# fredrikekre/PartitionedArrays.jl

Measured on AMD Instinct MI355X. Metric: SpMV+halo GB/s (frac of HBM peak), 3D Poisson 27-pt, 1/2/4/8 MI355X, higher is better.
Workload: dtype f64

## Files before the change

include/pa_hip.h:

```cpp
#ifndef PA_HIP_H
#define PA_HIP_H

#include <stdint.h>

#ifdef __cplusplus
extern "C" {
#endif

enum { PA_F32 = 0, PA_F64 = 1, PA_C64 = 2, PA_C128 = 3 };
enum { PA_REPLACE = 0, PA_ADD = 1 };

typedef struct pa_ctx pa_ctx;
typedef struct pa_index pa_index;
typedef struct pa_xchg pa_xchg;
typedef struct pa_vec pa_vec;
typedef struct pa_mat pa_mat;
typedef struct pa_coo pa_coo;
typedef struct pa_table pa_table;
typedef struct pa_event pa_event;

const char* pa_last_error(void);
int pa_version(void);
int pa_device_count(int* count);
int pa_tune(const char* key, int value, int* previous);
// ... 84 lines not shown
                  int* depth, int* result_flags);
int pa_vec_eval(pa_vec* y, const pa_index* y_idx, const pa_expr* prog, int nvec,
                const pa_vec* const v[], const pa_index* const v_idx[], int nscal,
                const void* scalars, const int* scalar_kinds, int all_lids);
int pa_reduce_expr_all(int n, int kind, const pa_expr* prog, int nvec,
                       const pa_vec* const v[], const pa_index* const v_idx[], int nscal,
                       const void* scalars, const int* scalar_kinds, void* result);

int pa_mat_from_csc(pa_ctx* ctx, int dtype, int index_bytes,
                    int64_t nrows_lids, int64_t ncols_lids,
                    const void* colptr, const void* rowval, const void* nzval,
                    const pa_index* rows, const pa_index* cols,
                    pa_mat** out);
int pa_mat_from_csr(pa_ctx* ctx, int dtype, int index_bytes, int Bi,
                    int64_t nrows_lids, int64_t ncols_lids,
                    const void* rowptr, const void* colval, const void* nzval,
                    const pa_index* rows, const pa_index* cols,
                    pa_mat** out);
int pa_mat_from_coo(pa_ctx* ctx, int dtype, int index_bytes, int ids_global,
                    int64_t nrows_lids, int64_t ncols_lids, int64_t ncoo,
                    const void* I, const void* J, const void* V,
                    const pa_index* rows, const pa_index* cols,
                    int64_t* csc_nnz, int64_t* colptr_out,
                    int64_t* rowval_out, pa_mat** out);
int pa_mat_from_coo_csr(pa_ctx* ctx, int dtype, int index_bytes, int ids_global, int Bi,
                        int64_t nrows_lids, int64_t ncols_lids, int64_t ncoo,
                        const void* I, const void* J, const void* V,
                        const pa_index* rows, const pa_index* cols, int64_t* nnz,
                        int64_t* rowptr_out, int64_t* colval_out, pa_mat** out);
int pa_mat_from_dcoo_csr(const pa_coo* coo, int ids_global, int Bi, int64_t nrows_lids,
                         int64_t ncols_lids, const pa_index* rows, const pa_index* cols,
                         int64_t* nnz, int64_t* rowptr_out, int64_t* colval_out,
                         pa_mat** out);
int pa_coo_create(pa_ctx* ctx, int dtype, int64_t n, const int64_t* I,
                  const int64_t* J, const void* V, pa_coo** out);
int pa_coo_destroy(pa_coo* coo);
int pa_coo_size(const pa_coo* coo, int64_t* n);
int pa_coo_download(const pa_coo* coo, int64_t* I, int64_t* J, void* V);
int pa_coo_assemble_all(int n, pa_coo* const coo[], const pa_index* const rows[],
                        pa_xchg* const rows_xchg[]);
int pa_coo_exchange_all(int n, pa_coo* const coo[], const pa_index* const rows[],
                        pa_xchg* const rows_xchg[]);
int pa_mat_from_dcoo(const pa_coo* coo, int ids_global, int64_t nrows_lids,
                     int64_t ncols_lids, const pa_index* rows,
                     const pa_index* cols, int64_t* csc_nnz,
                     int64_t* colptr_out, int64_t* rowval_out, pa_mat** out);
int pa_mat_set_values(pa_mat* A, const void* nzval);
int pa_mat_fillstored(pa_mat* A, const void* v);
int pa_mat_get_values(const pa_mat* A, void* nzval);
int pa_mat_scatter(pa_mat* A, pa_index* rows, pa_index* cols, int ids_kind,
                   int index_bytes, int op, int on_device, int64_t n,
                   const void* I, const void* J, const void* V);
int pa_mat_gather(const pa_mat* A, pa_index* rows, pa_index* cols, int ids_kind,
                  int index_bytes, int absent_zero, int on_device, int64_t n,
                  const void* I, const void* J, void* out);
int pa_mat_entry_info(const pa_mat* A, int64_t* entries, int64_t* bytes);
#define PA_NZ_OWNED_ROWS 0
#define PA_NZ_ALL_ROWS 1
int pa_mat_findnz(pa_mat* A, pa_index* rows, pa_index* cols, int which_rows, int ids_kind,
                  pa_coo** out);
int pa_mat_xchg_create(pa_mat* A, int32_t n_rcv, const int32_t* parts_rcv,
                       const int32_t* ptrs_rcv, const int64_t* k_rcv,
                       int32_t n_snd, const int32_t* parts_snd,
                       const int32_t* ptrs_snd, const int64_t* k_snd,
                       pa_xchg** out);
int pa_mat_exchange_all(int n, pa_mat* const A[], pa_xchg* const xg[],
                        int op, int reverse, int zero_sent);
int pa_mat_destroy(pa_mat* A);
int pa_mat_info(const pa_mat* A, int64_t* nrows_owned, int64_t* nnz_owned,
                int64_t* slots, int64_t* nslices, int64_t* nslices_interior);
int pa_mat_format_info(const pa_mat* A, int64_t* pattern_slices,
                       int64_t* regular_rows, int64_t* side_rows,
                       int64_t* side_slots);
int pa_mat_delta16_info(const pa_mat* A, int64_t* delta16_slices);
int pa_mat_triple_info(const pa_mat* A, int64_t* t_slices, int64_t* t_rows, int64_t* tri_slices,
                       int64_t* tri_rows);
int pa_mat_pair_info(const pa_mat* A, int64_t* pair_slices, int64_t* pair_rows);

int pa_mat_device_ptrs(const pa_mat* A, uint64_t out[8]);

int pa_mat_traffic(const pa_mat* A, int64_t* value_bytes, int64_t* index_bytes,
                   int64_t* meta_bytes);

int pa_mat_long_rows(const pa_mat* A, int64_t* n_long, int64_t* n_long_nnz);

int pa_spmv_all(int n, pa_mat* const A[], pa_vec* const y[],
                const pa_index* const y_idx[],
                pa_vec* const x[], const pa_index* const x_idx[],
                pa_xchg* const xg[], const void* alpha, const void* beta);

int pa_spmv_dot_all(int n, pa_mat* const A[], pa_vec* const y[],
                    const pa_index* const y_idx[],
                    pa_vec* const x[], const pa_index* const x_idx[],
                    pa_xchg* const xg[], const void* alpha, const void* beta,
                    void* dot_result);
int pa_cg_update_all(int n, pa_vec* const x[], pa_vec* const r[],
                     const pa_vec* const u[], const pa_vec* const c[],
                     const pa_index* const idx[], const void* alpha,
                     double* rnorm);

int pa_mat_diag(const pa_mat* A, const pa_index* rows, const pa_index* cols, pa_vec* d);
int pa_pcg_apply_all(int n, pa_vec* const c[], const pa_vec* const r[], const pa_vec* const d[], const pa_index* const idx[], void* rho);
int pa_pcg_update_all(int n, pa_vec* const x[], pa_vec* const r[], const pa_vec* const u[], pa_vec* const c[], const pa_vec* const d[], const pa_index* const idx[], const void* alpha, double* rnorm, void* rho);

int pa_cg_solve_all(int n, pa_mat* const A[], pa_vec* const x[],
                    const pa_vec* const b[], pa_vec* const u[],
                    pa_vec* const r[], pa_vec* const c[],
                    const pa_index* const idx[], pa_xchg* const xg[],
                    double reltol, double abstol, int64_t maxiter, int batch,
                    int64_t* iterations, double* residual, double* history);

typedef int (*pa_allreduce_max_fn)(float* v, int n, void* user);
int pa_cg_variant_agree(const float local_ms[2], pa_allreduce_max_fn fn, void* user, int* choice);
int pa_cg_fuse_agree(int local_can_fuse, pa_allreduce_max_fn fn, void* user, int* agreed);
int pa_mat_cg_choice(const pa_mat* A, int* choice);

int pa_exchange_all(int n, pa_vec* const v[], pa_xchg* const xg[],
                    const pa_index* const idx[], int op, int reverse,
                    int zero_ghosts);

int pa_exchange_all_async(int n, pa_vec* const v[], pa_xchg* const xg[],
                          const pa_index* const idx[], int op, int reverse,
                          int zero_ghosts, pa_event* const after[],
                          pa_event* done[]);
int pa_mat_exchange_all_async(int n, pa_mat* const A[], pa_xchg* const xg[],
                              int op, int reverse, int zero_sent,
                              pa_event* const after[], pa_event* done[]);
int pa_event_record(pa_ctx* ctx, pa_event** out);
int pa_event_query(const pa_event* ev, int* done);
int pa_event_wait(pa_event* ev);
int pa_ctx_wait_event(pa_ctx* ctx, const pa_event* ev);
int pa_event_destroy(pa_event* ev);

int pa_table_create(pa_ctx* ctx, int dtype, int64_t nrows, const int32_t* ptrs,
                    int ptrs_on_device, pa_table** out);
int pa_table_destroy(pa_table* t);
int pa_table_data(pa_table* t, pa_vec** data);
int pa_table_info(const pa_table* t, int64_t* nrows, int64_t* ndata);
int pa_table_ptrs(const pa_table* t, int32_t* ptrs);
int pa_table_exchange_all(int n, pa_table* const tables[], pa_xchg* const xg[],
                          int op, int reverse, int zero_sent);
int pa_table_exchange_all_async(int n, pa_table* const tables[], pa_xchg* const xg[],
                                int op, int reverse, int zero_sent,
                                pa_event* const after[], pa_event* done[]);

int pa_dot_all(int n, const pa_vec* const a[], const pa_index* const ia[],
               const pa_vec* const b[], const pa_index* const ib[],
               void* result);
int pa_norm2_all(int n, const pa_vec* const a[], const pa_index* const ia[],
                 void* result);
int pa_sum_all(int n, const pa_vec* const a[], const pa_index* const ia[],
               void* result);

int pa_mat_stencil(pa_ctx* ctx, int dtype, int kind, const int64_t gdims[3],
                   const int64_t box_lo[3], const int64_t box_n[3],
                   int64_t nlids_cols, const int32_t* shell_lid,
                   const double* coeffs, int ncoeffs, pa_mat** out);

int pa_ctx_set_timing(pa_ctx* ctx, int enable);
int pa_ctx_kernel_times(pa_ctx* ctx, float* interior_ms, float* halo_ms,
                        float* boundary_ms, int* count);
int pa_ctx_last_kernel_ms(pa_ctx* ctx, float* spmv_interior_ms,
                          float* spmv_boundary_ms);
int pa_ctx_span(pa_ctx* ctx, int stop);
int pa_ctx_span_ms(pa_ctx* ctx, float* ms);

// ... 5 lines not shown
```

partitionedarrays.jl_amd/_lib.py:

```python
from __future__ import annotations

import ctypes as C
import os

import numpy as np

_HERE = os.path.dirname(os.path.abspath(__file__))
LIB_PATH = os.environ.get("PA_HIP_LIB") or os.path.join(_HERE, "libpa_hip.so")

PA_F32, PA_F64, PA_C64, PA_C128 = 0, 1, 2, 3
PA_REPLACE, PA_ADD = 0, 1
TUNE_DROP = -(2 ** 31)
PA_BCAST_F64, PA_BCAST_C128 = 8, 16
PA_IDS_LOCAL, PA_IDS_GLOBAL = 0, 1
PA_SCATTER_ADD, PA_SCATTER_SET = 0, 1
PA_NZ_OWNED_ROWS, PA_NZ_ALL_ROWS = 0, 1

EXPR_MAX_OPS, EXPR_MAX_VECS, EXPR_MAX_SCALARS, EXPR_MAX_DEPTH = 32, 8, 8, 4
(OP_VEC, OP_SCAL, OP_ADD, OP_SUB, OP_MUL, OP_DIV, OP_NEG, OP_ABS, OP_ABS2, OP_CONJ,
 OP_LT, OP_LE, OP_GT, OP_GE, OP_EQ, OP_NE) = range(16)
EXPR_WIDE, EXPR_LREAL, EXPR_RREAL = 1, 2, 4
EXPR_SS, EXPR_SC, EXPR_CS, EXPR_RS = 0, 8, 16, 24
REDUCE_SUM, REDUCE_MAX, REDUCE_MIN = 0, 1, 2

# ... 50 lines not shown
    "pa_vec_upload": [_p, _p, C.c_int64],
    "pa_vec_download": [_p, _p, C.c_int64],
    "pa_vec_device_ptr": [_p, _p],
    "pa_vec_fill": [_p, _p],
    "pa_vec_copy": [_p, _p, _p, _p, C.c_int],
    "pa_vec_axpby": [_p, _p, _p, _p, C.c_int, C.c_int],
    "pa_vec_scatter": [_p, _p, C.c_int, C.c_int, C.c_int, C.c_int, C.c_int, C.c_int64, _p, _p],
    "pa_vec_gather": [_p, _p, C.c_int, C.c_int, C.c_int, C.c_int, C.c_int64, _p, _p],
    "pa_expr_check": [_p, C.c_int, C.c_int, C.c_int, C.POINTER(C.c_int), C.POINTER(C.c_int), C.POINTER(C.c_int)],
    "pa_vec_eval": [_p, _p, _p, C.c_int, C.POINTER(_p), C.POINTER(_p), C.c_int, _p, C.POINTER(C.c_int), C.c_int],
    "pa_reduce_expr_all": [C.c_int, C.c_int, _p, C.c_int, C.POINTER(_p), C.POINTER(_p), C.c_int, _p,
                           C.POINTER(C.c_int), _p],
    "pa_mat_from_csc": [_p, C.c_int, C.c_int, C.c_int64, C.c_int64, _p, _p, _p, _p, _p, C.POINTER(_p)],
    "pa_mat_from_csr": [_p, C.c_int, C.c_int, C.c_int, C.c_int64, C.c_int64, _p, _p, _p, _p, _p, C.POINTER(_p)],
    "pa_coo_create": [_p, C.c_int, C.c_int64, _i64p, _i64p, _p, C.POINTER(_p)],
    "pa_coo_destroy": [_p],
    "pa_coo_size": [_p, _i64p],
    "pa_coo_download": [_p, _i64p, _i64p, _p],
    "pa_coo_assemble_all": [C.c_int, C.POINTER(_p), C.POINTER(_p), C.POINTER(_p)],
    "pa_coo_exchange_all": [C.c_int, C.POINTER(_p), C.POINTER(_p), C.POINTER(_p)],
    "pa_mat_from_dcoo": [_p, C.c_int, C.c_int64, C.c_int64, _p, _p, _i64p, _i64p, _i64p, C.POINTER(_p)],
    "pa_mat_from_coo": [_p, C.c_int, C.c_int, C.c_int, C.c_int64, C.c_int64, C.c_int64, _p, _p, _p, _p, _p, _i64p,
                        _i64p, _i64p, C.POINTER(_p)],
    "pa_mat_from_coo_csr": [_p, C.c_int, C.c_int, C.c_int, C.c_int, C.c_int64, C.c_int64, C.c_int64, _p, _p, _p, _p,
                            _p, _i64p, _i64p, _i64p, C.POINTER(_p)],
    "pa_mat_from_dcoo_csr": [_p, C.c_int, C.c_int, C.c_int64, C.c_int64, _p, _p, _i64p, _i64p, _i64p,
                             C.POINTER(_p)],
    "pa_mat_fillstored": [_p, _p],
    "pa_index_set_gids": [_p, _i64p],
    "pa_add_gids": [_p, C.c_int64, _i64p, C.c_int64, _i64p, _i64p],
    "pa_index_to_lids": [_p, C.c_int64, _i64p],
    "pa_index_to_gids": [_p, C.c_int64, _i64p],
    "pa_mat_findnz": [_p, _p, _p, C.c_int, C.c_int, C.POINTER(_p)],
    "pa_mat_set_values": [_p, _p],
    "pa_mat_get_values": [_p, _p],
    "pa_mat_scatter": [_p, _p, _p, C.c_int, C.c_int, C.c_int, C.c_int, C.c_int64, _p, _p, _p],
    "pa_mat_gather": [_p, _p, _p, C.c_int, C.c_int, C.c_int, C.c_int, C.c_int64, _p, _p, _p],
    "pa_mat_entry_info": [_p, _i64p, _i64p],
    "pa_mat_xchg_create": [_p, C.c_int32, _i32p, _i32p, _i64p, C.c_int32, _i32p, _i32p, _i64p, C.POINTER(_p)],
    "pa_mat_exchange_all": [C.c_int, C.POINTER(_p), C.POINTER(_p), C.c_int, C.c_int, C.c_int],
    "pa_mat_destroy": [_p],
    "pa_mat_info": [_p, _i64p, _i64p, _i64p, _i64p, _i64p],
    "pa_mat_format_info": [_p, _i64p, _i64p, _i64p, _i64p],
    "pa_mat_delta16_info": [_p, _i64p],
    "pa_mat_triple_info": [_p, _i64p, _i64p, _i64p, _i64p],
    "pa_mat_pair_info": [_p, _i64p, _i64p],
    "pa_mat_long_rows": [_p, _i64p, _i64p],
    "pa_mat_stencil": [_p, C.c_int, C.c_int, _i64p, _i64p, _i64p, C.c_int64, _i32p, C.POINTER(C.c_double), C.c_int, C.POINTER(_p)],
    "pa_spmv_all": [C.c_int, C.POINTER(_p), C.POINTER(_p), C.POINTER(_p), C.POINTER(_p), C.POINTER(_p), C.POINTER(_p), _p, _p],
    "pa_spmv_dot_all": [C.c_int, C.POINTER(_p), C.POINTER(_p), C.POINTER(_p), C.POINTER(_p), C.POINTER(_p), C.POINTER(_p), _p, _p, _p],
    "pa_cg_update_all": [C.c_int, C.POINTER(_p), C.POINTER(_p), C.POINTER(_p), C.POINTER(_p), C.POINTER(_p), _p, C.POINTER(C.c_double)],
    "pa_mat_diag": [_p, _p, _p, _p],
    "pa_pcg_apply_all": [C.c_int, C.POINTER(_p), C.POINTER(_p), C.POINTER(_p), C.POINTER(_p), _p],
    "pa_pcg_update_all": [C.c_int, C.POINTER(_p), C.POINTER(_p), C.POINTER(_p), C.POINTER(_p), C.POINTER(_p),
                          C.POINTER(_p), _p, C.POINTER(C.c_double), _p],
    "pa_cg_solve_all": [C.c_int, C.POINTER(_p), C.POINTER(_p), C.POINTER(_p), C.POINTER(_p), C.POINTER(_p),
                        C.POINTER(_p), C.POINTER(_p), C.POINTER(_p), C.c_double, C.c_double, C.c_int64, C.c_int,
                        _i64p, C.POINTER(C.c_double), C.POINTER(C.c_double)],
    "pa_exchange_all": [C.c_int, C.POINTER(_p), C.POINTER(_p), C.POINTER(_p), C.c_int, C.c_int, C.c_int],
    "pa_exchange_all_async": [C.c_int, C.POINTER(_p), C.POINTER(_p), C.POINTER(_p), C.c_int, C.c_int, C.c_int,
                              C.POINTER(_p), C.POINTER(_p)],
    "pa_mat_exchange_all_async": [C.c_int, C.POINTER(_p), C.POINTER(_p), C.c_int, C.c_int, C.c_int, C.POINTER(_p),
                                  C.POINTER(_p)],
    "pa_table_create": [_p, C.c_int, C.c_int64, _p, C.c_int, C.POINTER(_p)],
    "pa_table_destroy": [_p],
    "pa_table_data": [_p, C.POINTER(_p)],
    "pa_table_info": [_p, _i64p, _i64p],
    "pa_table_ptrs": [_p, _i32p],
    "pa_table_exchange_all": [C.c_int, C.POINTER(_p), C.POINTER(_p), C.c_int, C.c_int, C.c_int],
    "pa_table_exchange_all_async": [C.c_int, C.POINTER(_p), C.POINTER(_p), C.c_int, C.c_int, C.c_int, C.POINTER(_p),
                                    C.POINTER(_p)],
    "pa_event_record": [_p, C.POINTER(_p)],
    "pa_event_query": [_p, C.POINTER(C.c_int)],
    "pa_event_wait": [_p],
    "pa_ctx_wait_event": [_p, _p],
    "pa_event_destroy": [_p],
    "pa_dot_all": [C.c_int, C.POINTER(_p), C.POINTER(_p), C.POINTER(_p), C.POINTER(_p), _p],
    "pa_norm2_all": [C.c_int, C.POINTER(_p), C.POINTER(_p), _p],
    "pa_sum_all": [C.c_int, C.POINTER(_p), C.POINTER(_p), _p],
    "pa_ctx_last_kernel_ms": [_p, C.POINTER(C.c_float), C.POINTER(C.c_float)],
    "pa_ctx_kernel_times": [_p, C.POINTER(C.c_float), C.POINTER(C.c_float), C.POINTER(C.c_float),
                            C.POINTER(C.c_int)],
    "pa_mat_traffic": [_p, _i64p, _i64p, _i64p],
    "pa_mat_device_ptrs": [_p, _p],
    "pa_ctx_span": [_p, C.c_int],
    "pa_ctx_span_ms": [_p, C.POINTER(C.c_float)],
    "pa_ctx_set_timing": [_p, C.c_int],
}

EXPORTED = sorted(list(_SIGS) + ["pa_last_error"])


class PAError(RuntimeError):
    pass


def _prepare_runtime():
    try:
        import torch
    except Exception:
        pass


def lib():
    global _lib
    if _lib is not None:
        return _lib
    if not os.path.exists(LIB_PATH):
        raise PAError(f"{LIB_PATH} not built: run `python -c 'import __graft_entry__ as g; g.build()'`")
    _prepare_runtime()
    L = C.CDLL(LIB_PATH)
    for name, args in _SIGS.items():
        if os.environ.get("PA_HIP_LIB") and not hasattr(L, name):
            continue
        f = getattr(L, name)
        f.argtypes = args
        f.restype = C.c_int
    L.pa_last_error.argtypes = []
    L.pa_last_error.restype = C.c_char_p
    _lib = L
    return L


def call(name, *args):
    L = lib()
    rc = getattr(L, name)(*args)
    if rc != 0:
        raise PAError(f"{name}: {L.pa_last_error().decode(errors='replace')}")


def device_count() -> int:
    n = C.c_int(0)
    call("pa_device_count", C.byref(n))
    return n.value


def tune(key: str, value: int) -> int:
    prev = C.c_int(0)
    call("pa_tune", key.encode(), int(value), C.byref(prev))
    return prev.value


def knob_selftest(nthreads: int = 4, iters: int = 2000) -> int:
    n = C.c_int(-1)
    call("pa_knob_selftest", int(nthreads), int(iters), C.byref(n))
    return n.value


ALLREDUCE_MAX_FN = C.CFUNCTYPE(C.c_int, C.POINTER(C.c_float), C.c_int, C.c_void_p)


def cg_variant_agree(local_ms, allreduce_max=None) -> int:
    ms = (C.c_float * 2)(*[float(v) for v in local_ms])
    cb = None
    if allreduce_max is not None:
        def _cb(v, n, _user):
            try:
                out = allreduce_max([v[i] for i in range(n)])
                for i in range(n):
                    v[i] = float(out[i])
                return 0
            except Exception:
                return 1
        cb = ALLREDUCE_MAX_FN(_cb)
    ch = C.c_int(-3)
    call("pa_cg_variant_agree", ms, C.cast(cb, C.c_void_p) if cb else None, None, C.byref(ch))
# ... 52 lines not shown
```

partitionedarrays.jl_amd/csrc/pa_api.cpp:

```cpp
#include <dlfcn.h>
#include <hip/hip_runtime.h>
#include <rccl/rccl.h>

#include <algorithm>
#include <chrono>
#include <cmath>
#include <cstdio>
#include <cstdlib>
#include <cstring>
#include <memory>
#include <numeric>
#include <string>
#include <unordered_map>
#include <atomic>
#include <condition_variable>
#include <functional>
#include <mutex>
#include <thread>
#include <vector>

#include "pa_internal.h"

namespace pa {

static thread_local std::string g_err;
void set_error(const std::string& msg) { g_err = msg; }

void launch_spmv_part(SliceKind kind, const SpmvPart& q, bool has_alpha, int bmode, const void* alpha,
                      const void* beta, hipStream_t st);
void launch_delta16(pa_mat* A, int64_t noids, const int32_t* kind, int32_t* ok, hipStream_t st);
void launch_pattern_detect(pa_mat* A, int64_t noids, int min_pct, int32_t* kind, int32_t* plen, int32_t* pat,
                           uint64_t* mask, int32_t* pghost, int32_t* nirreg, hipStream_t st);
void launch_side_len(pa_mat* A, int64_t n, const int32_t* rows, int32_t* len, int64_t noids,
                     int32_t* sghost, hipStream_t st);
void launch_side_fill(pa_mat* A, const int32_t* rows, const int32_t* len, hipStream_t st);
void launch_fold(int cplx, int nb, const void* in, void* scratch, void* out, unsigned* ticket, hipStream_t st);
void launch_fold_cg_alpha(int dtype, int nb, const void* in, void* scratch, void* out, unsigned* ticket,
                          CGState* cst, hipStream_t st);
void launch_fold_cg_step(int dtype, int nb, const void* in, void* scratch, void* out, unsigned* ticket,
                         CGState* cst, double* history, hipStream_t st);
void launch_cg_xr(int dtype, int64_t n, int64_t noids, const int32_t* own, void* x, void* r, const void* u,
                  const void* c, const void* alpha, const CGState* cst, double* part, int nb, hipStream_t st);
void launch_cg_xu(int dtype, int64_t n, void* x, void* u, const void* r, const CGState* cst, hipStream_t st);
void launch_cg_ghost(int dtype, int64_t lo, int64_t hi, const void* r, const void* uo, void* un, void* x,
                     const CGState* cst, hipStream_t st);
void launch_cg_alpha(int dtype, int P, const void* gathered, CGState* cst, hipStream_t st);
void launch_cg_step(int dtype, int P, const double* gathered, CGState* cst, double* history, hipStream_t st);
void launch_gather_ptrs(int P, const void* const* srcs, int accsz, void* out, hipStream_t st);
void launch_gather_scatter(int P, const void* const* srcs, int accsz, int nd, void* const* dsts, hipStream_t st);
const Knobs kDefaults = {
     223,  1,  1,  1,  1,
     65536,  2,  1,  0,  1,
     1,  0,  1,  0,  -1,  1,
     1,  1,  1,  0,  7,  1,
     0};
int coo_compress(int dtype, int index_bytes, int64_t m, int64_t ncols, int64_t n, const void* dI, const void* dJ,
                 const void* dV, int csr, int64_t* nu_out, DevBuf<int32_t>& crow, DevBuf<int32_t>& ccol,
                 DevBuf<void>& cval, DevBuf<int64_t>& colptr, hipStream_t st, hipError_t* err);
int coo_row_order(int64_t nu, const int32_t* crow, const int32_t* ccol, const int32_t* rl2o, const int32_t* cl2o,
                  int64_t nrows, int64_t noids_c, int64_t ncols, int H, DevBuf<uint64_t>& key2, DevBuf<int64_t>& idx2,
                  DevBuf<int64_t>& rowptr, DevBuf<int64_t>& gflag, DevBuf<int64_t>& grank, DevBuf<int32_t>& slen,
                  DevBuf<int32_t>& sghost, int64_t* nnz_out, int64_t* ngh_out, hipStream_t st, hipError_t* err);
void coo_slices(int64_t ns, int64_t nrows, int H, const int64_t* rowptr, const uint64_t* key2, int64_t ncols,
                int64_t noids_c, const int32_t* lidx, int32_t* slen, int32_t* sghost, hipStream_t st);
void coo_fill(int dtype, int64_t nnz, int64_t nu, const uint64_t* key2, const int64_t* idx2, const int64_t* rowptr,
              const int64_t* soff, int H, int R, int64_t ncols, const int32_t* crow, const int32_t* ccol,
              const void* cval, const int64_t* gflag, const int64_t* grank, int64_t slots, int32_t* col, void* val,
              int64_t* nz_slot, const int32_t* lidx, const int64_t* lptr, int32_t* lcol, int64_t long_off,
              int32_t* grc, hipStream_t st);
void launch_fill_i32(int64_t n, int32_t* a, int32_t v, hipStream_t st);
void launch_spmv_long(const pa_mat* A, const void* x, void* y, const int32_t* ymap, bool has_alpha, int bmode,
                      const void* alpha, const void* beta, void* dotp, int64_t dot_base, hipStream_t st);
int gid_table(int64_t n, const int64_t* d_lid_to_gid, DevBuf<uint64_t>& sgid, DevBuf<int64_t>& slid, hipStream_t st);
int gids_to_lids(int64_t n, int64_t* ids, const uint64_t* sgid, const int64_t* slid, int64_t nl, hipStream_t st);
int lids_to_gids(int64_t n, int64_t* ids, const int64_t* l2g, int64_t nl, hipStream_t st);
int coo_send_pack(bool to_ghosts, int dtype, const CooList& in, const uint64_t* sgid, const int64_t* slid, int64_t nl,
                  const std::vector<int32_t>& lid_to_ohid, const XchgSide& side, CooList* out,
                  std::vector<int64_t>* cnt, hipStream_t st);
int gids_first_touch(int64_t n, const int64_t* gids, const uint64_t* sgid, const int64_t* slid, int64_t nl,
                     DevBuf<int64_t>& out, int64_t* m_out, hipStream_t st);
void launch_pack(int dtype, int64_t n, const int32_t* lids, const void* v, void* buf,
                 hipStream_t st, hipEvent_t ev = nullptr);
void launch_unpack(int dtype, int64_t n, const int32_t* lids, const pa_combine_plan& plan, int op,
                   const void* buf, void* v, hipStream_t st);
void launch_pull(int dtype, int64_t n, const int32_t* lids, const pa_combine_plan& plan, int op, const int32_t* bid,
                 const int64_t* elem, const void* const* bases, void* v, hipStream_t st, hipEvent_t ev = nullptr);
void launch_fill(int dtype, int64_t n, int64_t base, const int32_t* map, void* v, const void* s,
                 hipStream_t st);
int launch_spmv_merged(int n, const SliceKind* kinds, const SpmvPart* parts, bool has_alpha, int bmode,
                       const void* alpha, const void* beta, pa_ctx* owner,
                       hipStream_t st);
void launch_spmv_group(SliceKind kind, int np, const SpmvPart* parts, bool has_alpha, int bmode, const void* alpha,
                       const void* beta, hipStream_t st);
void launch_pack_group(int dtype, const PackGroup& g, hipStream_t st);
void launch_pull_group(int dtype, const PullGroup& g, hipStream_t st);
void launch_copy(int dtype, int64_t n, const int32_t* dmap, void* d, const int32_t* smap,
                 const void* s, hipStream_t st);
void launch_axpby(int dtype, int64_t n, const int32_t* map, void* y, const void* x, const void* a,
                  int mode, hipStream_t st, int sk = 0);
void launch_reduce(int dtype, int kind, int64_t n, const int32_t* ma, const void* a,
                   const int32_t* mb, const void* b, void* partials, void* result,
                   unsigned* ticket, hipStream_t st);
void launch_stencil_count(const StencilGeom& g, const int32_t* shell, const double* coef,
                          int64_t nrows, int noids, int H, int32_t* slen, int32_t* sghost,
                          int32_t* err, hipStream_t st);
void launch_stencil_fill(const StencilGeom& g, const int32_t* shell, const double* coef,
                         int64_t nrows, int noids, pa_mat* A, int32_t* err, hipStream_t st);
void launch_probe(int copy, int unroll, int64_t n16, const void* a, void* b, int blocks, hipStream_t st);
void launch_invalid_config();
void launch_t_rowinfo(const pa_mat* A, int64_t n, const int32_t* rows, int64_t noids, int32_t* info, hipStream_t st);
void launch_t_pairinfo(const pa_mat* A, int64_t n, const int32_t* rows, int32_t* pairable, hipStream_t st);
void launch_u_fill(const pa_mat* A, hipStream_t st);
void launch_t_gbase(const pa_mat* A, int64_t noids, int32_t* ok, hipStream_t st);
void launch_t_fill(const pa_mat* A, int64_t noids, bool codes, hipStream_t st);
void launch_t_check(const pa_mat* A, unsigned* bad, hipStream_t st);
void launch_mat_diag(const pa_mat* A, const int32_t* own, void* d, int64_t nd, hipStream_t st);
void launch_pcg_apply(int dtype, int64_t n, int64_t noids, void* c, const void* r, const void* d, double* part,
                      int nb, hipStream_t st);
void launch_pcg_update(int dtype, int64_t n, int64_t noids, void* x, void* r, const void* u, void* c, const void* d,
                       const void* alpha, void* part, int nb, hipStream_t st);

}

using namespace pa;

#define PA_FAIL(msg)             \
  do {                           \
    pa::set_error(msg);          \
    return -1;                   \
  } while (0)

#define HIPC(expr)                                                                       \
  do {                                                                                   \
    hipError_t e_ = (expr);                                                              \
    if (e_ != hipSuccess) {                                                              \
      pa::set_error(std::string(#expr) + " failed: " + hipGetErrorString(e_));           \
      return -1;                                                                         \
    }                                                                                    \
  } while (0)

#define NCCLC(expr)                                                                      \
  do {                                                                                   \
    ncclResult_t r_ = (expr);                                                            \
    if (r_ != ncclSuccess) {                                                             \
      pa::set_error(std::string(#expr) + " failed: " + ncclGetErrorString(r_));          \
      return -1;                                                                         \
    }                                                                                    \
  } while (0)

#define CHECK_ARG(cond, msg) \
  do {                       \
    if (!(cond)) PA_FAIL(msg); \
  } while (0)

namespace {

template <typename T>
int dev_upload(T** dptr, const std::vector<T>& h) {
  *dptr = nullptr;
  if (h.empty()) return 0;
  HIPC(hipMalloc((void**)dptr, h.size() * sizeof(T)));
  HIPC(hipMemcpy(*dptr, h.data(), h.size() * sizeof(T), hipMemcpyHostToDevice));
  return 0;
}

void dev_free(void* p) {
  if (p) (void)hipFree(p);
}

bool valid_dtype(int dt) { return dt == PA_F32 || dt == PA_F64 || dt == PA_C64 || dt == PA_C128; }

bool scalar_is(int dt, const void* s, double re) {
  switch (dt) {
    case PA_F32: return *(const float*)s == (float)re;
    case PA_F64: return *(const double*)s == re;
    case PA_C64: { const float* f = (const float*)s; return f[0] == (float)re && f[1] == 0.f; }
    case PA_C128: { const double* d = (const double*)s; return d[0] == re && d[1] == 0.0; }
  }
  return false;
}

int build_plan(const std::vector<int32_t>& lids, pa_combine_plan* plan) {
  const int64_t n = (int64_t)lids.size();
  std::vector<int32_t> order(n);
  std::iota(order.begin(), order.end(), 0);
  std::stable_sort(order.begin(), order.end(), [&](int32_t a, int32_t b) { return lids[a] < lids[b]; });
  std::vector<int32_t> target, ptr{0}, pos;
  pos.reserve(n);
  for (int64_t i = 0; i < n; ++i) {
    const int32_t l = lids[order[i]];
    if (target.empty() || target.back() != l) {
      if (!target.empty()) ptr.push_back((int32_t)pos.size());
      target.push_back(l);
    }
    pos.push_back(order[i]);
// ... 443 lines not shown
    A->main.col16.reset();
    A->main.gbase.reset();
    return 0;
  }
  HIPC(hipMemcpyAsync(A->d_kind, kind.data(), ns * 4, hipMemcpyHostToDevice, st));
  if (A->nz_map && A->R == 4 && remap_nz_interleaved(A, kind, st)) return -1;
  if (knobs().spmv_tri16 && A->R <= 2 && build_triple_sell(A, kind, noids)) return -1;
  return 0;
}

int upload_set(SliceSet& S, const std::vector<int32_t>& in, const std::vector<int32_t>& bnd) {
  S.n_int = (int64_t)in.size();
  S.n_bnd = (int64_t)bnd.size();
  HIPC(S.d_int.upload(in));
  HIPC(S.d_bnd.upload(bnd));
  return 0;
}

int build_slice_lists(pa_mat* A, const std::vector<int32_t>& kind, const Detected& D, std::vector<int32_t>* side) {
  const int64_t ns = A->main.nslices;
  const int W = A->H / 64;
  std::vector<int32_t> pint, pbnd, xint, xbnd, dint, dbnd;
  A->maxlen_pat = A->maxlen_pm_int = A->maxlen_d16 = 0;
  for (int64_t s = 0; s < ns; ++s) {
    const bool g = D.pghost[s] != 0;
    switch (kind[s]) {
      case kBkPattern:
        (g ? pbnd : pint).push_back((int32_t)s);
        A->maxlen_pat = std::max(A->maxlen_pat, (int)A->h_plen[s]);
        break;
      case kBkDelta16:
        (g ? dbnd : dint).push_back((int32_t)s);
        A->maxlen_d16 = std::max(A->maxlen_d16, (int)A->h_slen[s]);
        break;
      case kBkInt32:
        (g ? xbnd : xint).push_back((int32_t)s);
        A->maxlen_pm_int = std::max(A->maxlen_pm_int, (int)A->h_slen[s]);
        break;
      default: break;
    }
    if (kind[s] != kBkPattern) continue;
    ++A->npattern_slices;
    const int64_t nvalid = std::min<int64_t>(A->H, A->main.nrows - s * A->H);
    for (int64_t i = 0; i < nvalid; ++i) {
      if ((D.mask[s * W + i / 64] >> (i & 63)) & 1ull) ++A->nregular_rows;
      else if (!is_long_row(A, s * A->H + i)) side->push_back((int32_t)(s * A->H + i));
    }
  }
  A->h_kind = kind;
  return upload_set(A->sl_pat, pint, pbnd) || upload_set(A->sl_i32, xint, xbnd) || upload_set(A->sl_d16, dint, dbnd);
}

int build_side_sell(pa_mat* A, const std::vector<int32_t>& rows, int64_t noids) {
  Sell& S = A->side;
  S.nrows = (int64_t)rows.size();
  if (S.nrows == 0) return 0;
  hipStream_t st = A->ctx->s_main;
  const int64_t H = A->H, nss = (S.nrows + H - 1) / H;
  std::vector<int32_t> rl;
  {
    HIPC(S.rowmap.upload(rows));
    DevBuf<int32_t> d_sghost;
    HIPC(S.rowlen.alloc(S.nrows));
    HIPC(d_sghost.alloc(nss));
    HIPC(hipMemsetAsync(d_sghost, 0, nss * 4, st));
    launch_side_len(A, S.nrows, S.rowmap, S.rowlen, noids, d_sghost, st);
    HIPC(hipGetLastError());
    HIPC(download(rl, S.rowlen.p, S.nrows, st));
    HIPC(hipStreamSynchronize(st));
  }
  std::vector<int32_t> slen(nss, 0);
  for (int64_t i = 0; i < S.nrows; ++i) slen[i / H] = std::max(slen[i / H], rl[i]);
  const std::vector<int64_t> soff = sell_offsets(S, slen, (int)H);
  HIPC(S.off.upload(soff));
  HIPC(S.len.upload(slen));
  HIPC(S.col.alloc(std::max<int64_t>(S.slots, 1)));
  HIPC(S.val.alloc(std::max<int64_t>(S.slots, 1) * dtype_size(A->dtype)));
  launch_side_fill(A, S.rowmap, S.rowlen, st);
  HIPC(hipGetLastError());
  HIPC(hipStreamSynchronize(st));
  return 0;
}

int finalize_pattern(pa_mat* A, int kmax, int64_t noids, bool retry_r2) {
  A->kmax = std::max(kmax, 1);
  if (A->main.nslices == 0) return 0;
  Detected D;
  if (detect_patterns(A, noids, &D)) return -1;
  if (retry_r2 && prefers_r2(A, D.kind)) return kPreferR2;
  std::vector<int32_t> kind = D.kind, side;
  if (dedup_patterns(A, kind) || encode_delta16(A, noids, kind) || build_slice_lists(A, kind, D, &side) ||
      build_side_sell(A, side, noids))
    return -1;
  A->has_pat = true;
  return 0;
}

struct LocalSet {
  std::vector<int> pos_of_part;
  int find(int part) const {
    return (part >= 1 && part < (int)pos_of_part.size()) ? pos_of_part[part] : -1;
  }
};

template <typename H>
LocalSet local_set(int n, H* const* hs) {
  LocalSet L;
  int maxp = 0;
  bool all_comm = true;
  for (int i = 0; i < n; ++i) {
    const pa_ctx* c = hs[i]->ctx;
    maxp = std::max(maxp, c->nparts);
    all_comm = all_comm && c->comm != nullptr && (c->halo_rccl || knobs().halo_transport == 1);
  }
  L.pos_of_part.assign(maxp + 1, -1);
  if (all_comm) return L;
  for (int i = 0; i < n; ++i) L.pos_of_part[hs[i]->ctx->part] = i;
  return L;
}

int peer_segment(const pa_xchg* Q, int dir, int part, int64_t cnt, int* m) {
  const XchgSide& q = Q->from(dir);
  const auto it = std::find(q.parts.begin(), q.parts.end(), part);
  CHECK_ARG(it != q.parts.end(), "exchanger mismatch: a receiver lists a sender that does not send to it");
  *m = (int)(it - q.parts.begin());
  CHECK_ARG(cnt < 0 || cnt == q.ptrs[*m + 1] - q.ptrs[*m],
            "exchanger mismatch: segment lengths differ (SequentialBackend.jl:187)");
  return 0;
}

const char* side_name(int dir) { return dir ? "parts_rcv" : "parts_snd"; }

uint64_t g_xchg_next_id = 1;

int build_pull(int i, int n, pa_xchg* const xg[], const LocalSet& L, int dtype, int dir, bool alt = false) {
  pa_xchg* X = xg[i];
  pa_ctx* c = X->ctx;
  pa_pull& P = alt ? X->pull_alt : X->pull[dir];
  auto sender_buf = [&](const pa_xchg* Q) -> void* { return alt ? Q->buf_snd2 : Q->from(dir).buf; };
  const auto& prcv = X->into(dir).parts;
  const auto& orcv = X->into(dir).ptrs;
  void* own = X->into(dir).buf;
  std::vector<const void*> key;
  key.push_back((const void*)(intptr_t)dtype_size(dtype));
  for (int32_t q : prcv) {
    const int j = L.find(q);
    key.push_back(j >= 0 ? (const void*)(uintptr_t)xg[j]->id : nullptr);
    key.push_back(j >= 0 ? sender_buf(xg[j]) : own);
  }
  if (P.built && P.key == key) return 0;
  HIPC(hipSetDevice(c->device));
  P = pa_pull{};
  P.built = true;
  P.key = key;
  std::vector<void*> bases;
  auto base_id = [&](void* b) {
    for (size_t t = 0; t < bases.size(); ++t)
      if (bases[t] == b) return (int32_t)t;
    bases.push_back(b);
    return (int32_t)(bases.size() - 1);
  };
  const int64_t nslots = orcv.empty() ? 0 : orcv.back();
  std::vector<int32_t> bid(nslots);
  std::vector<int64_t> elem(nslots);
  for (size_t k = 0; k < prcv.size(); ++k) {
    const int j = L.find(prcv[k]);
    const int64_t cnt = orcv[k + 1] - orcv[k];
    if (j < 0) {
      const int32_t b = base_id(own);
      for (int64_t t = 0; t < cnt; ++t) { bid[orcv[k] + t] = b; elem[orcv[k] + t] = orcv[k] + t; }
      continue;
    }
    pa_xchg* Q = xg[j];
    const auto& qo = Q->from(dir).ptrs;
    int m = -1;
// ... 388 lines not shown
  int64_t lo, hi;
  int64_t mask;
  const char* help;
};
const Knob kKnobs[] = {
    {"spmv_flags", &Knobs::spmv_flags, nullptr, 0, 0xff, 0xff,
     "spmv_flags: bit 0 = non-temporal streams, bit 1 = pattern and triple-SELL slices' one-load descriptor, "
     "bit 2 = 16 B x runs (pattern rows), bit 3 = masked tail batch, bit 4 = identity slice lists dropped, "
     "bit 5 = non-temporal y stores, bit 6 = short-row kernels (launches whose rows have <= 8 entries), "
     "bit 7 = the Float64 short-row tail launch at 7 entries and 7 waves per SIMD (rows <= 7 entries)"},
    {"long_rows_exact", &Knobs::long_exact, nullptr, 0, 1, 0,
     "long_rows_exact: 1 = reference summation order, 0 = lane-strided tree (1e-12)"},
    {"halo_pull", &Knobs::halo_pull, nullptr, 0, 1, 0,
     "halo_pull: 1 = receivers read the senders' buffers (one kernel), 0 = staging copies"},
    {"spmv_delta16", &Knobs::spmv_delta16, nullptr, 0, 1, 0,
     "spmv_delta16: 1 = int32-column slices whose columns fit 16-bit codes store those (matrices built "
     "afterwards; default), 0 = int32 column ids"},
    {"spmv_merge", &Knobs::spmv_merge, nullptr, 0, 1, 0,
     "spmv_merge: 1 = mul! without a halo in flight (one part, or parts of one stream pair with the direct "
     "pull) runs every slice kind of every part as one launch (default), 0 = one launch per kind"},
    {"spmv_merge_max", nullptr, &Knobs::spmv_merge_max, 0, INT32_MAX, 0,
     "spmv_merge_max: one part with more slices than this runs one launch per kind (0: always merge)"},
    {"cg_fuse", &Knobs::cg_fuse, nullptr, 0, 2, 0,
     "cg_fuse: 1 = the device CG computes u = r .+ beta.*u inside the SpMV, 0 = a separate sweep, "
     "2 = auto (default: one batch of each, then the faster; all parts in one process, else the sweep)"},
    {"halo_direct", &Knobs::halo_direct, nullptr, 0, 1, 0,
     "halo_direct: 1 = mul! over parts sharing a stream pair reads the ghosts straight from the owners' x "
     "on the compute stream (default), 0 = pack + pull on the comm stream"},
    {"halo_transport", &Knobs::halo_transport, nullptr, 0, 1, 0,
     "halo_transport: 0 = parts of this process by device reads/copies, 1 = RCCL send/recv for every part "
     "with a communicator (pa_comm_init_all)"},
    {"spmv_group", &Knobs::spmv_group, nullptr, 0, 1, 0,
     "spmv_group: 1 = one launch per phase for parts sharing a stream pair, 0 = per part"},
    {"spmv_format", &Knobs::spmv_format, nullptr, 0, 1, 0, "spmv_format: 0 = int32 columns, 1 = pattern slices"},
    {"pattern_min_regular", &Knobs::pattern_min_pct, nullptr, 0, 100, 0,
     "pattern_min_regular: a slice becomes a pattern slice when at least this % of its rows follow its pattern "
     "(matrices built afterwards); 0 = auto (default): 70 for 128-row slices, 50 for Float32's 256-row slices"},
    {"issue_threads", &Knobs::issue_threads, nullptr, 0, 2, 0,
     "issue_threads: a call over parts with their own stream pairs is issued from host threads, one part "
     "per thread: 1 = when the parts span several devices (default), 2 = always, 0 = never (the calling "
     "thread, one part after the other)"},
    {"spmv_tri16", &Knobs::spmv_tri16, nullptr, 0, 1, 0,
     "spmv_tri16: the delta16 slices' rows re-sliced into the triple SELL (rows of consecutive column triples "
     "keep one 16-bit code per triple; matrices built afterwards): 1 = slices of 1-2 rows per lane (Float64, "
     "ComplexF32, ComplexF64, Float32 with f32_rows 2; default), 0 = never"},
    {"f32_rows", &Knobs::f32_rows, nullptr, 0, 4, 6,
     "f32_rows: Float32 SELL rows per lane (matrices built afterwards): 4 = 16 B value packs in 256-row "
     "slices, 2 = 8 B packs in 128-row slices (the Float64 geometry; delta16 rows then take the triple "
     "SELL), 0 = auto (default): 4, rebuilt with 2 when fewer than 80 % of the slices are pattern slices "
     "(C5 F32 -7 %, FE27 256^3 F32 +14 % with 2, profiles/r05/af/)"},
    {"spmv_tri_pack", &Knobs::tri_pack, nullptr, 0, 7, 0,
     "spmv_tri_pack: triple-SELL slices of 2 rows per lane (matrices built afterwards): bit 2 = pair slices "
     "(all element types): rows a, a + 1 whose columns differ by one, entry for entry, share one lane, one "
     "code and one x run per triple (C5 F32 -2.4 %, F64 -1 %, profiles/r06/u/); bit 0 = Float32 pair slices: "
     "a triple's values as one 16 B pack (entries 0 and 1 of both rows) and one 8 B pack (entry 2) per lane "
     "(two loads instead of three); bit 1: unused since r06/aa (the Float32 tri slices' code packs); 7 = "
     "default, 0 = none"},
    {"spmv_uniform", &Knobs::spmv_uniform, nullptr, 0, 1, 0,
     "spmv_uniform: Float64 pattern slices whose patterns (<= 7 entries) fit one union U (FD7; matrices built "
     "afterwards): 1 = a copy of their values at slice * H * |U| in U's entry order, so the short-row tail "
     "launch issues its value and x loads before the slice descriptor arrives (default), 0 = off"},
    {"spmv_side_tail", &Knobs::side_tail, nullptr, 0, 1, 0,
     "spmv_side_tail: per-kind launches without a halo in flight (big single parts): 1 = the side rows (<= 8 "
     "entries) run as the trailing waves of the pattern launch (default: FE27 256^3 -0.4 %, profiles/r05/o/), "
     "0 = a launch of their own after it"},
    {"spmv_tri_order", &Knobs::tri_order, nullptr, 0, 1, 0,
     "spmv_tri_order: the triple SELL's row order (matrices built afterwards): 1 = the other rows first "
     "(their slower waves start early, the launch ends on uniform triple slices; default: C5 F64 -1 %, "
     "Float32 triples -4..-7 %, profiles/r05/n/), 0 = rows of column triples first"},
    {"halo_barrier", &Knobs::halo_barrier, nullptr, 0, 2, 0,
     "halo_barrier: mul! over parts with their own stream pairs and local neighbours (one process driving "
     "several GPUs): 1 = one pack barrier event per call and double-buffered send buffers (default), 2 = the "
     "same with each part's pull on its compute stream after its interior slices (one runtime call less per "
     "part), 0 = per-neighbour event waits before every pack and every pull"},
    {"spmv_xcd_chunk", &Knobs::spmv_xcd_chunk, nullptr, -1, 64, 0,
     "spmv_xcd_chunk: the SpMV launches' workgroups in runs of C consecutive blocks per XCD (C > 0; the x lines "
     "of neighbouring slices shared in one L2), 0 = the hardware's round robin, -1 = auto (default): per-kind "
     "launches (big single parts) take C = the pattern's reach in blocks / 8, so that a block's z-neighbour "
     "plane runs on its XCD (FE27 256^3 F64: C = 16, -1.0..-1.2 %, profiles/r05/q,r/), merged launches keep "
     "the round robin (C2: C = 4 +1.4 %, r05/k/)"},
    {"scatter_wide", &Knobs::scatter_wide, nullptr, 0, 1, 0,
     "scatter_wide: the ordered vector scatter (pa_vec_scatter) sorts 0 = 32-bit keys and payloads when the "
     "part's local ids and the entries fit them (default), 1 = always the 64-bit ones (A/B, tests)"},
    {"fault_inject", &Knobs::fault_inject, nullptr, 0, 1, 0,
     "fault_inject: 1 = every job of a threaded issue (IssuePool) also issues an invalid kernel launch (tests "
     "of the error path; test_exception.jl's role), 0 = off (default)"},
};
constexpr int kNumKnobs = (int)(sizeof(kKnobs) / sizeof(kKnobs[0]));
static_assert(kNumKnobs <= pa_ctx::kMaxKnobs, "pa_ctx::over too small");

std::mutex g_knob_mu;
Knobs g_knob_defaults = kDefaults;
thread_local const Knobs* t_knobs = nullptr;
thread_local Knobs t_knob_snapshot;

int knob_find(const char* key) {
  for (int i = 0; i < kNumKnobs; ++i)
    if (!std::strcmp(key, kKnobs[i].key)) return i;
  pa::set_error(std::string("pa_tune: unknown key ") + key);
  return -1;
}
int knob_index(const char* key, int64_t value) {
  const int i = knob_find(key);
  if (i < 0) return -1;
  const Knob& k = kKnobs[i];
  if (value < k.lo || value > k.hi || (k.mask != 0 && (value & ~k.mask) != 0)) {
    pa::set_error(k.help);
    return -2;
  }
  return i;
}
int64_t knob_get(const Knobs& K, int i) { return kKnobs[i].slot ? (int64_t)(K.*kKnobs[i].slot) : K.*kKnobs[i].slot64; }
void knob_set(Knobs& K, int i, int64_t v) {
  if (kKnobs[i].slot) K.*kKnobs[i].slot = (int)v;
  else K.*kKnobs[i].slot64 = v;
}
}

namespace pa {
const Knobs& knobs() {
  if (t_knobs) return *t_knobs;
  std::lock_guard<std::mutex> g(g_knob_mu);
  t_knob_snapshot = g_knob_defaults;
  return t_knob_snapshot;
}
KnobBind::KnobBind(const Knobs* k) : prev(t_knobs) { t_knobs = k; }
KnobBind::~KnobBind() { t_knobs = prev; }
thread_local int t_force_f32_rows = 0;
int f32_rows_knob() { return t_force_f32_rows ? t_force_f32_rows : (knobs().f32_rows == 2 ? 2 : 4); }
struct ForceF32Rows {
  int prev;
  explicit ForceF32Rows(int r) : prev(t_force_f32_rows) { t_force_f32_rows = r; }
  ~ForceF32Rows() { t_force_f32_rows = prev; }
};
}

TuneScope::TuneScope(const pa_ctx* c) : prev(t_knobs) {
  if (prev) {
    k = *prev;
  } else {
    std::lock_guard<std::mutex> g(g_knob_mu);
    k = g_knob_defaults;
  }
  if (c && !prev)
    for (int i = 0; i < kNumKnobs; ++i)
      if (c->has_over[i]) knob_set(k, i, c->over[i]);
  t_knobs = &k;
}
TuneScope::~TuneScope() { t_knobs = prev; }

extern "C" {

int pa_tune(const char* key, int value, int* previous) {
  CHECK_ARG(key, "null key");
  const int i = knob_index(key, value);
  if (i < 0) return -1;
  std::lock_guard<std::mutex> g(g_knob_mu);
  if (previous) *previous = (int)std::min<int64_t>(knob_get(g_knob_defaults, i), INT32_MAX);
  knob_set(g_knob_defaults, i, value);
  return 0;
}

int pa_ctx_tune(pa_ctx* c, const char* key, int value, int* previous) {
  CHECK_ARG(c && key, "null argument");
  const int i = value == PA_TUNE_DROP ? knob_find(key) : knob_index(key, value);
  if (i < 0) return -1;
// ... 1374 lines not shown
  HIPC(hipSetDevice(c->device));
  auto C = std::make_unique<pa_coo>();
  C->ctx = c;
  C->dtype = dtype;
  C->l.n = n;
  if (n > 0) {
    const size_t S = dtype_size(dtype);
    HIPC(C->l.I.alloc(n));
    HIPC(C->l.J.alloc(n));
    HIPC(C->l.V.alloc(n * S));
    HIPC(hipMemcpy(C->l.I, I, n * 8, hipMemcpyHostToDevice));
    HIPC(hipMemcpy(C->l.J, J, n * 8, hipMemcpyHostToDevice));
    HIPC(hipMemcpy(C->l.V, V, n * S, hipMemcpyHostToDevice));
  }
  *out = C.release();
  return 0;
}

int pa_coo_destroy(pa_coo* C) {
  if (!C) return 0;
  (void)hipSetDevice(C->ctx->device);
  (void)hipStreamSynchronize(C->ctx->s_main);
  delete C;
  return 0;
}

int pa_coo_size(const pa_coo* C, int64_t* n) {
  CHECK_ARG(C && n, "null argument");
  *n = C->l.n;
  return 0;
}

int pa_coo_download(const pa_coo* C, int64_t* I, int64_t* J, void* V) {
  CHECK_ARG(C && (C->l.n == 0 || (I && J && V)), "null argument");
  const int64_t n = C->l.n;
  if (n == 0) return 0;
  HIPC(hipSetDevice(C->ctx->device));
  HIPC(hipStreamSynchronize(C->ctx->s_main));
  HIPC(hipMemcpy(I, C->l.I, n * 8, hipMemcpyDeviceToHost));
  HIPC(hipMemcpy(J, C->l.J, n * 8, hipMemcpyDeviceToHost));
  HIPC(hipMemcpy(V, C->l.V, n * dtype_size(C->dtype), hipMemcpyDeviceToHost));
  return 0;
}

int pa_coo_assemble_all(int n, pa_coo* const coo[], const pa_index* const rows[], pa_xchg* const xg[]) {
  return coo_send_all(false, n, coo, rows, xg);
}

int pa_coo_exchange_all(int n, pa_coo* const coo[], const pa_index* const rows[], pa_xchg* const xg[]) {
  return coo_send_all(true, n, coo, rows, xg);
}

static int load_nz_map(const pa_mat* cA) {
  CHECK_ARG(cA->nz_map, "matrix was not built from a CSC pattern");
  pa_mat* A = const_cast<pa_mat*>(cA);
  if (A->d_nz_slot) {
    HIPC(hipSetDevice(A->ctx->device));
    HIPC(hipStreamSynchronize(A->ctx->s_main));
    A->h_nz_slot.resize(A->csc_nnz);
    HIPC(hipMemcpy(A->h_nz_slot.data(), A->d_nz_slot, A->csc_nnz * 8, hipMemcpyDeviceToHost));
    A->d_nz_slot.reset();
  }
  return 0;
}

static inline int64_t nz_index(const pa_mat* A, int64_t p) {
  const int64_t s = A->h_nz_slot[p];
  return s >= 0 ? s : A->main.slots - s - 1;
}

static int refresh_side(pa_mat* A, hipStream_t st) {
  if (A->side.nrows > 0) {
    launch_side_fill(A, A->side.rowmap, A->side.rowlen, st);
    HIPC(hipGetLastError());
  }
  if (A->tri.nrows > 0) {
    launch_t_fill(A, 0, false, st);
    HIPC(hipGetLastError());
  }
  if (A->uni.val) {
    launch_u_fill(A, st);
    HIPC(hipGetLastError());
  }
  return 0;
}

int pa_mat_set_values(pa_mat* A, const void* nzval) {
  CHECK_ARG(A && nzval, "null argument");
  if (load_nz_map(A)) return -1;
  HIPC(hipSetDevice(A->ctx->device));
  const size_t S = dtype_size(A->dtype);
  const int64_t nv = nvals(A);
  std::vector<unsigned char> hval(nv * S, 0);
  for (int64_t p = 0; p < A->csc_nnz; ++p)
    std::memcpy(&hval[nz_index(A, p) * S], (const unsigned char*)nzval + p * S, S);
  HIPC(hipStreamSynchronize(A->ctx->s_main));
  if (nv) HIPC(hipMemcpy(A->main.val, hval.data(), nv * S, hipMemcpyHostToDevice));
  if (refresh_side(A, A->ctx->s_main)) return -1;
  HIPC(hipStreamSynchronize(A->ctx->s_main));
  return 0;
}

int pa_mat_fillstored(pa_mat* A, const void* v) {
  CHECK_ARG(A && v, "null argument");
  HIPC(hipSetDevice(A->ctx->device));
  const int64_t nv = nvals(A);
  if (nv) launch_fill(A->dtype, nv, 0, nullptr, A->main.val, v, A->ctx->s_main);
  HIPC(hipGetLastError());
  if (refresh_side(A, A->ctx->s_main)) return -1;
  return 0;
}

int pa_mat_get_values(const pa_mat* A, void* nzval) {
  CHECK_ARG(A && nzval, "null argument");
  if (load_nz_map(A)) return -1;
  HIPC(hipSetDevice(A->ctx->device));
  const size_t S = dtype_size(A->dtype);
  const int64_t nv = nvals(A);
  std::vector<unsigned char> hval(nv * S, 0);
  HIPC(hipStreamSynchronize(A->ctx->s_comm));
  HIPC(hipStreamSynchronize(A->ctx->s_main));
  if (nv) HIPC(hipMemcpy(hval.data(), A->main.val, nv * S, hipMemcpyDeviceToHost));
  for (int64_t p = 0; p < A->csc_nnz; ++p)
    std::memcpy((unsigned char*)nzval + p * S, &hval[nz_index(A, p) * S], S);
  return 0;
}


static int mat_value_ids(const std::string& w, const pa_mat* cA, const pa_index* rows, const pa_index* cols,
                         bool global, int index_bytes, bool absent_zero, bool stored, int64_t n, const void* dI,
                         const void* dJ, DevBuf<int64_t>& vidx) {
  pa_mat* A = const_cast<pa_mat*>(cA);
  hipStream_t st = A->ctx->s_main;
  CHECK_ARG(A->has_entries || mat_entry_table(A, rows, st) == 0, w + "building the entry table failed");
  HIPC(vidx.alloc(n));
  return ids_rc_check(w, mat_entry_ids(A, rows, cols, global, index_bytes, absent_zero, stored, n, dI, dJ, vidx, st),
                      global, w);
}

int pa_mat_scatter(pa_mat* A, pa_index* rows, pa_index* cols, int ids_kind, int index_bytes, int op, int on_device,
                   int64_t n, const void* I, const void* J, const void* V) {
  const std::string w = "pa_mat_scatter: ";
  CHECK_ARG(op == PA_SCATTER_ADD || op == PA_SCATTER_SET, w + "op must be PA_SCATTER_ADD or PA_SCATTER_SET");
  if (ids_scalar_check(w, ids_kind, index_bytes, n) ||
      mat_handle_check(w, A, rows, cols, n == 0 || (I && J && V), ids_kind))
    return -1;
  if (n == 0) return 0;
  pa_ctx* c = A->ctx;
  TuneScope ts(c);
  HIPC(hipSetDevice(c->device));
  const bool global = ids_kind == PA_IDS_GLOBAL;
  const size_t ibytes = (size_t)n * index_bytes;
  Staged sI, sJ, sV;
  DevBuf<int64_t> vidx;
  if (sI.in(on_device, I, ibytes, c->s_main) || sJ.in(on_device, J, ibytes, c->s_main) ||
      sV.in(on_device, V, (size_t)n * dtype_size(A->dtype), c->s_main))
    return -1;
  if (mat_value_ids(w, A, rows, cols, global, index_bytes, false, true, n, sI.dev, sJ.dev, vidx)) return -1;
  const int64_t nv = nvals(A);
  const int rc = vec_scatter(A->dtype, nv, A->main.val, false, 8, op == PA_SCATTER_SET, false, scatter_wide(nv, n), n,
                             vidx.p, sV.dev, nullptr, nullptr, c->s_main);
  CHECK_ARG(rc == 0, w + "device pass failed");
  return refresh_side(A, c->s_main);
}

int pa_mat_gather(const pa_mat* A, pa_index* rows, pa_index* cols, int ids_kind, int index_bytes, int absent_zero,
// ... 76 lines not shown
    vs[i].ctx = A[i]->ctx;
    vs[i].dtype = A[i]->dtype;
    vs[i].n = nvals(A[i]);
    vs[i].d = A[i]->main.val;
    vp[i] = &vs[i];
  }
  if (pa_exchange_all(n, vp.data(), xg, nullptr, op, reverse, 0)) return -1;
  for (int i = 0; i < n; ++i) {
    pa_ctx* c = A[i]->ctx;
    HIPC(hipSetDevice(c->device));
    if (zero_sent) {
      unsigned char z[16] = {0};
      const XchgSide& sent = xg[i]->from(reverse ? 1 : 0);
      launch_fill(A[i]->dtype, sent.n, 0, sent.lids, A[i]->main.val, z, c->s_main);
    }
    if (refresh_side(A[i], c->s_main)) return -1;
  }
  HIPC(hipGetLastError());
  return 0;
}

int pa_mat_destroy(pa_mat* A) {
  if (!A) return 0;
  (void)hipSetDevice(A->ctx->device);
  (void)hipStreamSynchronize(A->ctx->s_main);
  delete A;
  return 0;
}

int pa_mat_format_info(const pa_mat* A, int64_t* pattern_slices, int64_t* regular_rows,
                       int64_t* side_rows, int64_t* side_slots) {
  CHECK_ARG(A, "null matrix");
  if (pattern_slices) *pattern_slices = A->npattern_slices;
  if (regular_rows) *regular_rows = A->nregular_rows;
  if (side_rows) *side_rows = A->side.nrows;
  if (side_slots) *side_slots = A->side.slots;
  return 0;
}

int pa_mat_delta16_info(const pa_mat* A, int64_t* delta16_slices) {
  CHECK_ARG(A, "null matrix");
  if (delta16_slices) *delta16_slices = A->sl_d16.n_int + A->sl_d16.n_bnd;
  return 0;
}

int pa_mat_pair_info(const pa_mat* A, int64_t* pair_slices, int64_t* pair_rows) {
  CHECK_ARG(A, "null matrix");
  if (pair_slices) *pair_slices = A->tri.pair_slices;
  if (pair_rows) *pair_rows = A->tri.pair_rows;
  return 0;
}

int pa_mat_triple_info(const pa_mat* A, int64_t* t_slices, int64_t* t_rows, int64_t* tri_slices,
                       int64_t* tri_rows) {
  CHECK_ARG(A, "null matrix");
  if (t_slices) *t_slices = A->tri.nslices;
  if (t_rows) *t_rows = A->tri.nrows;
  if (tri_slices) *tri_slices = A->tri.tri_slices;
  if (tri_rows) *tri_rows = A->tri.tri_rows;
  return 0;
}

int pa_mat_long_rows(const pa_mat* A, int64_t* n_long, int64_t* n_long_nnz) {
  CHECK_ARG(A, "null matrix");
  if (n_long) *n_long = A->n_long;
  if (n_long_nnz) *n_long_nnz = A->n_lnz;
  return 0;
}

int pa_mat_device_ptrs(const pa_mat* A, uint64_t out[8]) {
  CHECK_ARG(A && out, "null argument");
  const void* p[8] = {A->main.val, A->main.col, A->main.off, A->d_plen, A->d_pat, A->d_mask, A->side.val, A->side.col};
  for (int i = 0; i < 8; ++i) out[i] = (uint64_t)(uintptr_t)p[i];
  return 0;
}

int pa_mat_traffic(const pa_mat* A, int64_t* value_bytes, int64_t* index_bytes, int64_t* meta_bytes) {
  CHECK_ARG(A, "null matrix");
  TuneScope ts(A->ctx);
  const int64_t S = (int64_t)dtype_size(A->dtype), H = A->H, W = H / 64;
  const bool pat = pattern_layout(A);
  const bool split = A->sl_all.d_bnd != nullptr;
  int64_t v = 0, ix = 0, m = 0;
  for (int64_t s = 0; s < A->main.nslices; ++s) {
    const int kd = pat ? A->h_kind[s] : kBkInt32;
    if (kd == kBkPattern) {
      v += (int64_t)(A->uni.val ? A->uni.K : A->h_plen[s]) * H * S;
      m += std::max<int64_t>(W * 8 + 8 + 4, 4 * desc_words(A->R)) + 4;
    } else if (kd == kBkDelta16) {
      v += (int64_t)A->h_slen[s] * H * S;
      ix += (int64_t)A->h_slen[s] * H * 2;
      m += 8 + 4 + 4 + 4;
    } else if (kd == kBkMoved) {
    } else {
      v += (int64_t)A->h_slen[s] * H * S;
      ix += (int64_t)A->h_slen[s] * H * 4;
      m += 8 + 4 + ((pat || split) ? 4 : 0);
    }
  }
  if (pat) {
    m += A->npatterns * A->kmax * 4;
    v += A->side.slots * S;
    ix += A->side.slots * 4 + A->side.nrows * 4;
    m += A->side.nslices * 12;
    v += A->tri.slots * S;
    ix += A->tri.code_slots * 2 + A->tri.nrows * 4;
    m += A->tri.nslices * (8 + 4 + 4 + 4);
  }
  v += A->n_lnz * S;
  ix += A->n_lnz * 4;
  m += A->n_long * 16;
  if (value_bytes) *value_bytes = v;
  if (index_bytes) *index_bytes = ix;
  if (meta_bytes) *meta_bytes = m;
  return 0;
}

int pa_mat_info(const pa_mat* A, int64_t* nrows, int64_t* nnz, int64_t* slots, int64_t* nslices,
                int64_t* nslices_int) {
  CHECK_ARG(A, "null matrix");
  if (nrows) *nrows = A->main.nrows;
  if (nnz) *nnz = A->nnz;
  if (slots) *slots = A->main.slots;
  if (nslices) *nslices = A->main.nslices;
  if (nslices_int) *nslices_int = A->sl_all.n_int;
  return 0;
}

constexpr int kMaxTimed = 1024;

struct CGFuse {
  std::vector<const void*> u_old;
  std::vector<void*> u_new, xacc;
  std::vector<CGState*> st;
};

static void cg_ghosts(const CGFuse* fz, int i, const pa_mat* A, const pa_vec* r, hipStream_t st) {
  if (!fz || r->n <= A->main.nrows) return;
  launch_cg_ghost(A->dtype, A->main.nrows, r->n, r->d, fz->u_old[i], fz->u_new[i], fz->xacc[i], fz->st[i], st);
}

enum SlicePhase { kInterior, kBoundary, kWhole };
struct SliceWork {
  SliceKind kind;
  int64_t nwork;
  const int32_t* list;
};
struct SliceList {
  SliceWork w[8];
  int n = 0;
  void add(SliceKind kind, int64_t nwork, const int32_t* list) { w[n++] = SliceWork{kind, nwork, list}; }
  const SliceWork* begin() const { return w; }
  const SliceWork* end() const { return w + n; }
};

static SliceList slice_list(const pa_mat* A, SlicePhase phase) {
  SliceList L;
  const bool in = phase != kBoundary, bnd = phase != kInterior;
  if (pattern_layout(A)) {
    const std::pair<SliceKind, const SliceSet*> sets[] = {
        {kPattern, &A->sl_pat}, {kInt32, &A->sl_i32}, {kDelta16, &A->sl_d16}};
    if (in)
      for (const auto& [k, S] : sets) L.add(k, S->n_int, S->d_int);
    if (bnd) {
      for (const auto& [k, S] : sets) L.add(k, S->n_bnd, S->d_bnd);
      L.add(kSide, A->side.nslices, nullptr);
    }
    if (phase == kWhole) L.add(kTriple, A->tri.nslices, nullptr);
    else if (in) L.add(kTriple, A->tri.list.n_int, A->tri.list.d_int);
    else L.add(kTriple, A->tri.list.n_bnd, A->tri.list.d_bnd);
  } else if (A->sl_all.d_bnd) {
    if (in) L.add(kInt32, A->sl_all.n_int, A->sl_all.d_int);
    if (bnd) L.add(kInt32, A->sl_all.n_bnd, A->sl_all.d_bnd);
  } else if (in) {
    L.add(kInt32, A->main.nslices, nullptr);
  }
  return L;
}

struct SpmvCall {
  int n;
  pa_mat* const* A;
  pa_vec* const* y;
  const pa_index* const* y_idx;
  pa_vec* const* x;
  pa_xchg* const* xg;
  bool any_x;
  int dt;
  bool has_alpha;
  int bmode;
  const void* alpha;
  const void* beta;
  std::vector<void*> dotp;
  bool want_dot;
  CGState* const* dot_tail;
  std::vector<hipEvent_t*> tslot;
  const CGFuse* fz;
  bool halo_first;

  const int32_t* ymap(int i) const { return y_idx[i]->own_contig ? nullptr : y_idx[i]->d_oid_to_lid; }

  SpmvPart part(int i, int64_t nwork, const int32_t* list) const {
    SpmvPart q{nwork, list, A[i], x[i]->d, y[i]->d, ymap(i), dotp[i]};
    if (fz) {
      q.xu = fz->u_old[i];
      q.un = fz->u_new[i];
      q.xacc = fz->xacc[i];
      q.cg = fz->st[i];
// ... 1742 lines not shown
```

partitionedarrays.jl_amd/csrc/pa_internal.h:

```cpp
#pragma once
#include <hip/hip_runtime.h>
#include <cstdint>
#include <memory>
#include <string>
#include <type_traits>
#include <vector>

#include "../../include/pa_hip.h"

namespace pa {

struct alignas(8) c64 {
  float re, im;
};
struct alignas(16) c128 {
  double re, im;
};

__host__ __device__ inline c64 operator+(c64 a, c64 b) { return {a.re + b.re, a.im + b.im}; }
__host__ __device__ inline c64 operator-(c64 a, c64 b) { return {a.re - b.re, a.im - b.im}; }
__host__ __device__ inline c64 operator*(c64 a, c64 b) {
  return {a.re * b.re - a.im * b.im, a.re * b.im + a.im * b.re};
}
__host__ __device__ inline c128 operator+(c128 a, c128 b) { return {a.re + b.re, a.im + b.im}; }
// ... 213 lines not shown
  int nvec;
  const void* v[PA_EXPR_MAX_VECS];
  const int32_t* map[PA_EXPR_MAX_VECS];
  c128 scal[PA_EXPR_MAX_SCALARS];
};
void launch_expr_store(int dtype, int64_t n, const ExprArgs& a, void* y, const int32_t* ymap, bool fast,
                       hipStream_t st);
void launch_expr_reduce(int dtype, int kind, int64_t n, const ExprArgs& a, bool fast, void* partials,
                        void* result, unsigned* ticket, hipStream_t st);

struct StencilGeom {
  int64_t N[3];
  int64_t lo[3];
  int64_t n[3];
  int kind;
};

}

struct pa_ctx {
  struct StreamRefs { int n = 1; };
  StreamRefs* stream_refs = nullptr;
  int device = 0;
  int part = 1;
  int nparts = 1;
  hipStream_t s_main = nullptr;
  hipStream_t s_comm = nullptr;
  void* comm = nullptr;
  bool halo_rccl = false;
  std::shared_ptr<void> comm_owner;
  std::shared_ptr<const std::vector<int>> rank_of_part;
  int peer_rank(int q) const { return rank_of_part ? (*rank_of_part)[q - 1] : q - 1; }
  int64_t rccl_bytes_sent = 0, rccl_bytes_recv = 0;
  void* d_partials = nullptr;
  void* d_fold = nullptr;
  void* d_result = nullptr;
  void* d_gather = nullptr;
  unsigned* d_ticket = nullptr;
  void* h_pinned = nullptr;
  bool timing = false;
  std::vector<hipEvent_t> tev;
  int tn = 0;
  hipEvent_t span_ev[2] = {nullptr, nullptr};
  hipEvent_t ev_packed = nullptr;
  hipEvent_t ev_recvd = nullptr;
  hipEvent_t ev_barrier = nullptr;
  std::vector<std::pair<std::vector<void*>, void**>> bases_cache;
  std::vector<std::pair<std::vector<char>, void*>> merged_cache;
  static constexpr int kMaxKnobs = 24;
  bool has_over[kMaxKnobs] = {};
  int64_t over[kMaxKnobs] = {};
};

struct pa_event {
  int device = 0;
  hipEvent_t ev[2] = {nullptr, nullptr};
};

namespace pa {
struct Knobs {
  int spmv_flags;
  int long_exact;
  int halo_pull;
  int spmv_delta16;
  int spmv_merge;
  int64_t spmv_merge_max;
  int cg_fuse;
  int halo_direct;
  int halo_transport;
  int spmv_group;
  int spmv_format;
  int pattern_min_pct;
  int issue_threads;
  int fault_inject;
  int spmv_xcd_chunk;
  int spmv_tri16;
  int halo_barrier;
  int tri_order;
  int side_tail;
  int f32_rows;
  int tri_pack;
  int spmv_uniform;
  int scatter_wide;
};
const Knobs& knobs();
struct KnobBind {
  explicit KnobBind(const Knobs* k);
  ~KnobBind();
  const Knobs* prev;
};
}

struct TuneScope {
  explicit TuneScope(const pa_ctx* c);
  ~TuneScope();
  TuneScope(const TuneScope&) = delete;
  TuneScope& operator=(const TuneScope&) = delete;
  pa::Knobs k;
  const pa::Knobs* prev;
};

namespace pa {
template <typename T>
struct DevBuf {
  T* p = nullptr;
  DevBuf() = default;
  DevBuf(DevBuf&& o) noexcept : p(o.p) { o.p = nullptr; }
  DevBuf& operator=(DevBuf&& o) noexcept {
    if (this != &o) adopt(o.p), o.p = nullptr;
    return *this;
  }
  DevBuf(const DevBuf&) = delete;
  DevBuf& operator=(const DevBuf&) = delete;
  ~DevBuf() { reset(); }
  void reset() { adopt(nullptr); }
  void adopt(T* q) {
    if (p) (void)hipFree(p);
    p = q;
  }
  hipError_t alloc(size_t n) {
    reset();
    return hipMalloc((void**)&p, n * sizeof(std::conditional_t<std::is_void<T>::value, char, T>));
  }
  template <typename U>
  hipError_t upload(const std::vector<U>& h) {
    static_assert(std::is_same<U, T>::value, "element type");
    reset();
    if (h.empty()) return hipSuccess;
    const hipError_t e = alloc(h.size());
    return e != hipSuccess ? e : hipMemcpy(p, h.data(), h.size() * sizeof(U), hipMemcpyHostToDevice);
  }
  operator T*() const { return p; }
  template <typename U>
  explicit operator U*() const { return (U*)p; }
};
template <typename T>
inline hipError_t download(std::vector<T>& h, const T* d, size_t n, hipStream_t st) {
  h.resize(n);
  return hipMemcpyAsync(h.data(), d, n * sizeof(T), hipMemcpyDeviceToHost, st);
}
}

struct pa_index {
  pa_ctx* ctx = nullptr;
  uint64_t id = 0;
  int64_t nlids = 0, noids = 0, nhids = 0;
  bool own_contig = true;
  bool ghost_contig = true;
  pa::DevBuf<int32_t> d_oid_to_lid;
  pa::DevBuf<int32_t> d_hid_to_lid;
  std::vector<int32_t> h_oid_to_lid;
  std::vector<int32_t> h_hid_to_lid;
  std::vector<int32_t> h_lid_to_ohid;
  pa::DevBuf<uint64_t> d_sgid;
  pa::DevBuf<int64_t> d_slid;
  pa::DevBuf<int64_t> d_lid_to_gid;
  bool has_gids = false;
};

struct pa_combine_plan {
  int64_t ntargets = 0;
  bool unique = true;
  pa::DevBuf<int32_t> d_target;
  pa::DevBuf<int32_t> d_ptr;
  pa::DevBuf<int32_t> d_pos;
};
// ... 37 lines not shown
  bool snd_in_rcv = false;
  uint64_t own_key = 0;
  bool rcv_owned = false;
  pa::XchgSide rcv, snd;
  pa::XchgSide& into(int dir) { return dir ? snd : rcv; }
  const pa::XchgSide& into(int dir) const { return dir ? snd : rcv; }
  pa::XchgSide& from(int dir) { return into(1 - dir); }
  const pa::XchgSide& from(int dir) const { return into(1 - dir); }
  int64_t max_lid = -1;
  pa::DevBuf<void> buf_snd2;
  pa_pull pull_alt;
  uint64_t fast_key = 0, fast_seq = 0;
  int fast_parity = 0;
};

constexpr size_t kVecPad = 64;

struct pa_coo {
  pa_ctx* ctx = nullptr;
  int dtype = PA_F64;
  pa::CooList l;
};

struct pa_vec {
  pa_ctx* ctx = nullptr;
  int dtype = PA_F64;
  int64_t n = 0;
  void* d = nullptr;
  pa::DevBuf<void> base;
};

struct pa_table {
  pa_ctx* ctx = nullptr;
  int dtype = PA_F64;
  int64_t nrows = 0, ndata = 0;
  pa::DevBuf<int32_t> t;
  pa_vec* data = nullptr;
  std::vector<std::pair<uint64_t, std::unique_ptr<pa_xchg>>> plans;
};

namespace pa {
hipError_t table_ptrs(int64_t nrows, const int32_t* d_ptrs1, int32_t* t, int* bad, int64_t* ndata, hipStream_t st);
int table_expand_side(const XchgSide& in, const int32_t* t, XchgSide* out, int64_t* total, hipStream_t st,
                      hipError_t* err);
}

constexpr int desc_words(int R) { return R <= 2 ? 8 : 16; }

namespace pa {
enum BuildKind : int32_t { kBkInt32 = 0, kBkPattern = 1, kBkDelta16 = 3, kBkMoved = 5 };

struct Sell {
  int64_t nrows = 0, nslices = 0;
  int64_t slots = 0;
  int maxlen = INT32_MAX;
  DevBuf<int64_t> off;
  DevBuf<int32_t> len;
  DevBuf<int32_t> col;
  DevBuf<uint16_t> col16;
  DevBuf<int32_t> gbase;
  DevBuf<void> val;
  DevBuf<int32_t> rowmap;
  DevBuf<int32_t> rowlen;
};
struct SliceSet {
  int64_t n_int = 0, n_bnd = 0;
  DevBuf<int32_t> d_int, d_bnd;
};
struct TripleSell : Sell {
  SliceSet list;
  DevBuf<int64_t> src;
  DevBuf<int32_t> desc;
  int pack = 0;
  int64_t tri_slices = 0, tri_rows = 0, code_slots = 0;
  int64_t pair_slices = 0, pair_rows = 0;
  std::vector<int32_t> h_len;
};
struct UniformRows {
  DevBuf<void> val;
  DevBuf<int32_t> emap;
  int K = 0;
  int32_t pat[8] = {0, 0, 0, 0, 0, 0, 0, 0};
};
}

struct pa_mat {
  pa_ctx* ctx = nullptr;
  int dtype = PA_F64;
  int cg_fuse_choice = -1;
  int R = 2;
  int H = 128;
  int64_t ncols_lids = 0;
  int64_t nnz = 0;
  bool csr = false;
  pa::Sell main;
  pa::SliceSet sl_all;
  std::vector<int32_t> h_slen, h_kind, h_plen;
  std::vector<int64_t> h_nz_slot;
  pa::DevBuf<int64_t> d_nz_slot;
  bool nz_map = false;
  int64_t csc_nnz = 0;
  int64_t n_gnz = 0;
  int64_t n_long = 0, n_lnz = 0, long_off = 0;
  pa::DevBuf<int32_t> d_long_row;
  pa::DevBuf<int64_t> d_long_ptr;
  pa::DevBuf<int32_t> d_long_col;
  pa::DevBuf<int32_t> d_sflags;
  pa::DevBuf<uint64_t> d_lmask;
  std::vector<int32_t> h_long_rows;
  int64_t n_lchunks = 0;
  pa::DevBuf<int64_t> d_lchunk_start;
  pa::DevBuf<int64_t> d_lrow_chunk;
  pa::DevBuf<void> d_lpart;

  bool has_pat = false;
  int kmax = 0;
  pa::DevBuf<int32_t> d_kind;
  pa::DevBuf<int32_t> d_pdesc;
  pa::DevBuf<int32_t> d_plen;
  pa::DevBuf<int32_t> d_pat;
  int64_t npatterns = 0;
  int xcd_auto = 0;
  pa::DevBuf<uint64_t> d_mask;
  int64_t npattern_slices = 0, nregular_rows = 0;
  pa::SliceSet sl_pat, sl_i32, sl_d16;
  int maxlen_pat = INT32_MAX, maxlen_pm_int = INT32_MAX, maxlen_d16 = INT32_MAX;
  pa::Sell side;
  pa::TripleSell tri;
  pa::UniformRows uni;
  pa::DevBuf<void> d_dotp;

  int64_t nrows_lids = 0;
  pa::DevBuf<int32_t> d_ghost_rc;
  bool has_entries = false;
  int64_t n_entries = 0;
  pa::DevBuf<uint64_t> d_ekey;
  pa::DevBuf<int64_t> d_eidx;
};

namespace pa {
inline bool pattern_layout(const pa_mat* A) { return knobs().spmv_format == 1 && A->has_pat; }

inline int64_t dot_base(const pa_mat* A, SliceKind k) {
  return k == kSide ? A->main.nslices : k == kTriple ? A->main.nslices + A->side.nslices : 0;
}
inline int64_t long_dot_base(const pa_mat* A) {
  return pattern_layout(A) ? dot_base(A, kTriple) + A->tri.nslices : A->main.nslices;
}

int mat_entry_table(pa_mat* A, const pa_index* rows, hipStream_t st);
int mat_entry_ids(const pa_mat* A, const pa_index* rows, const pa_index* cols, bool global, int index_bytes,
                  bool absent_zero, bool stored, int64_t n, const void* I, const void* J, int64_t* vidx,
                  hipStream_t st);
int mat_findnz(const pa_mat* A, const pa_index* rows, const pa_index* cols, bool owned_only, bool global,
               CooList& out, hipStream_t st);
}
```

partitionedarrays.jl_amd/csrc/pa_spmv.hip:

```cpp
#include "pa_internal.h"

#include <cstddef>

#include <algorithm>
#include <cstring>
#include <type_traits>

#if defined(PA_SPMV_DT)
#define PA_DT_DEFINE 0
#else
#define PA_DT_DEFINE 1
#endif
#define PA_CAT2(a, b) a##b
#define PA_CAT(a, b) PA_CAT2(a, b)

namespace pa {

template <typename T, int R>
struct alignas(sizeof(T) * R) Pack {
  T v[R];
};
template <int R>
struct alignas(4 * R) IPack {
  int32_t c[R];
};
template <int R>
struct alignas(2 * R) S16Pack {
  uint16_t c[R];
};

enum { SPMV_NT = 1, SPMV_DESC = 2 , SPMV_XPAIR = 4, SPMV_TAILB = 8, SPMV_IDLIST = 16, SPMV_YNT = 32, SPMV_SHORT = 64,
       SPMV_SHORT7 = 128 ,
       SPMV_PRODA = 256 ,
       SPMV_TPACK = 512  };

typedef unsigned int spmv_u32x4 __attribute__((ext_vector_type(4)));
static_assert((SPMV_NT | SPMV_DESC | SPMV_XPAIR | SPMV_TAILB | SPMV_IDLIST | SPMV_SHORT | SPMV_SHORT7) == 223,
              "kDefaults.spmv_flags");
template <int R>
constexpr int kDescWords = desc_words(R);

#if defined(__HIP_DEVICE_COMPILE__)
#define PA_GLB __attribute__((address_space(1)))
#else
#define PA_GLB
#endif

template <int BYTES> struct RawOf;
template <> struct RawOf<2> { typedef unsigned short type; };
template <> struct RawOf<4> { typedef unsigned int type; };
template <> struct RawOf<8> { typedef unsigned int type __attribute__((ext_vector_type(2))); };
template <> struct RawOf<16> { typedef unsigned int type __attribute__((ext_vector_type(4))); };

template <bool NT, typename V>
__device__ __forceinline__ V ld(const V* p) {
  typedef typename RawOf<sizeof(V)>::type Raw;
  Raw r;
  if (NT) r = __builtin_nontemporal_load(reinterpret_cast<const Raw*>(p));
  else r = *reinterpret_cast<const Raw*>(p);
  V v;
  __builtin_memcpy(&v, &r, sizeof(V));
  return v;
}

template <typename T>
struct SpmvArgs {
  int64_t nwork;
  const PA_GLB int32_t* list;
  const PA_GLB int64_t* soff;
  const PA_GLB int32_t* slen;
  const PA_GLB int32_t* col;
  const PA_GLB T* val;
  const PA_GLB int32_t* pat;
  const PA_GLB uint64_t* mask;
  int kmax;
  const PA_GLB int32_t* rowmap;
  int64_t nrows;
  const PA_GLB T* x;
  int64_t nx;
  PA_GLB T* y;
  const PA_GLB int32_t* ymap;
  T alpha, beta;
  int flags;
  const PA_GLB T* dotu;
  void* dotp;
  int64_t dot_base;
  const PA_GLB int32_t* sflags;
  const PA_GLB uint64_t* lmask;
  int maxlen;
  const PA_GLB uint16_t* col16;
  const PA_GLB int32_t* gbase;
  const PA_GLB int32_t* ilv;
  const PA_GLB T* xu;
  PA_GLB T* un;
  PA_GLB T* xacc;
  const PA_GLB CGState* cg;
  int xcd_chunk;
  const PA_GLB int32_t* desc;
  const PA_GLB T* uval;
  int uK;
  int32_t upat[8];
};

template <typename T> struct DAcc { using type = double; };
template <> struct DAcc<c64> { using type = c128; };
template <> struct DAcc<c128> { using type = c128; };
__device__ inline double dacc(float a) { return (double)a; }
__device__ inline double dacc(double a) { return a; }
__device__ inline c128 dacc(c64 a) { return c128{(double)a.re, (double)a.im}; }
__device__ inline c128 dacc(c128 a) { return a; }
__device__ inline double shfl_down_acc(double v, int d) { return __shfl_down(v, d, 64); }
__device__ inline c128 shfl_down_acc(c128 v, int d) {
  return c128{__shfl_down(v.re, d, 64), __shfl_down(v.im, d, 64)};
}

__device__ __forceinline__ float pick(bool c, float a, float b) { return c ? a : b; }
__device__ __forceinline__ double pick(bool c, double a, double b) { return c ? a : b; }
__device__ __forceinline__ c64 pick(bool c, c64 a, c64 b) { return c64{c ? a.re : b.re, c ? a.im : b.im}; }
__device__ __forceinline__ c128 pick(bool c, c128 a, c128 b) { return c128{c ? a.re : b.re, c ? a.im : b.im}; }

typedef unsigned int u4a __attribute__((ext_vector_type(4))) __attribute__((aligned(4)));
typedef unsigned int u2r __attribute__((ext_vector_type(2))) __attribute__((aligned(4)));
template <typename T, int R>
__device__ __forceinline__ Pack<T, R> ld_xrun(const T* p) {
  Pack<T, R> v;
  if constexpr (sizeof(Pack<T, R>) == 8) {
    const u2r r = *reinterpret_cast<const u2r*>(p);
    __builtin_memcpy(&v, &r, 8);
  } else {
    static_assert(sizeof(Pack<T, R>) == 16, "16 B runs");
    const u4a r = *reinterpret_cast<const u4a*>(p);
    __builtin_memcpy(&v, &r, 16);
  }
  return v;
}

typedef unsigned int u3a __attribute__((ext_vector_type(3))) __attribute__((aligned(4)));
typedef unsigned int u2a __attribute__((ext_vector_type(2))) __attribute__((aligned(4)));
template <typename T>
__device__ __forceinline__ void ld_xtrip(const T* p, T (&o)[3]) {
  if constexpr (sizeof(T) == 4) {
    const u3a r = *reinterpret_cast<const u3a*>(p);
    __builtin_memcpy(&o[0], &r, 12);
  } else if constexpr (sizeof(T) == 8) {
    const u4a r = *reinterpret_cast<const u4a*>(p);
    const u2a q = *reinterpret_cast<const u2a*>(p + 2);
    __builtin_memcpy(&o[0], &r, 16);
    __builtin_memcpy(&o[2], &q, 8);
  } else {
#pragma unroll
    for (int j = 0; j < 3; ++j) o[j] = p[j];
  }
}

template <typename T>
__device__ __forceinline__ void ld_xquad(const T* p, T (&o)[4]) {
  if constexpr (sizeof(T) == 4) {
    const u4a r = *reinterpret_cast<const u4a*>(p);
    __builtin_memcpy(&o[0], &r, 16);
  } else if constexpr (sizeof(T) == 8) {
    const u4a r0 = *reinterpret_cast<const u4a*>(p);
    const u4a r1 = *reinterpret_cast<const u4a*>(p + 2);
    __builtin_memcpy(&o[0], &r0, 16);
    __builtin_memcpy(&o[2], &r1, 16);
  } else {
#pragma unroll
    for (int j = 0; j < 4; ++j) o[j] = p[j];
  }
}

template <typename T, bool XV>
struct XSrc {
  const T* __restrict__ x;
  __device__ __forceinline__ T get(int64_t j) const { return x[j]; }
  __device__ __forceinline__ void quad(int64_t j, T (&o)[4]) const { ld_xquad<T>(x + j, o); }
  template <int R>
  __device__ __forceinline__ Pack<T, R> run(int64_t j) const { return ld_xrun<T, R>(x + j); }
  __device__ __forceinline__ void trip(int64_t j, T (&o)[3]) const { ld_xtrip<T>(x + j, o); }
};
template <typename T>
struct XSrc<T, true> {
  const T* __restrict__ r;
  const T* __restrict__ u;
  double b;
// ... 333 lines not shown
    q[0] = ld<NT>(&cp[t * 64]);
#pragma unroll
    for (int u = 0; u < 3; ++u) v[u] = ld<NT>(&vp[(3 * t + u) * 64]);
    step(q, v, std::integral_constant<int, 1>{});
  }
}

template <typename T, bool ALPHA, typename XS, bool TP, int NB, bool FULL>
__device__ __forceinline__ void pair_batch(T (&acc)[2], const uint16_t* __restrict__ cs,
                                           const Pack<T, 2>* __restrict__ vp, int t, int ntri, const XS& x, T alpha,
                                           bool pf, int32_t rowa, int32_t gb, bool packs) {
  constexpr int R = 2, NQ = NB / 4;
  const int lane = threadIdx.x % 64;
  uint16_t q[NB];
  if (FULL && packs) {
    const uint16_t* __restrict__ cb = cs + (int64_t)t * 64;
#pragma unroll
    for (int h = 0; h < NQ; ++h) {
      const S16Pack<4> q4 = ld<true>(reinterpret_cast<const S16Pack<4>*>(cb + h * 4 * 64) + lane);
#pragma unroll
      for (int i = 0; i < 4; ++i) q[4 * h + i] = q4.c[i];
    }
#pragma unroll
    for (int u = 4 * NQ; u < NB; ++u) q[u] = ld<true>(reinterpret_cast<const S16Pack<1>*>(cb + u * 64) + lane).c[0];
  } else {
#pragma unroll
    for (int u = 0; u < NB; ++u)
      q[u] = ld<true>(reinterpret_cast<const S16Pack<1>*>(cs + (int64_t)(FULL ? t + u : min(t + u, ntri - 1)) * 64) +
                      lane).c[0];
  }
  Pack<T, R> v[3 * NB];
  const Pack<T, R>* __restrict__ vb = vp - lane;
#pragma unroll
  for (int u = 0; u < NB; ++u) {
    const int tu = FULL ? t + u : min(t + u, ntri - 1);
    if constexpr (TP) {
      const Pack<T, R>* tb = vb + (int64_t)tu * 3 * 64;
      const Pack<T, 2 * R> p01 = ld<true>(reinterpret_cast<const Pack<T, 2 * R>*>(tb) + lane);
#pragma unroll
      for (int r = 0; r < R; ++r) {
        v[3 * u].v[r] = p01.v[r];
        v[3 * u + 1].v[r] = p01.v[R + r];
      }
      v[3 * u + 2] = ld<true>(tb + 2 * 64 + lane);
    } else {
#pragma unroll
      for (int j = 0; j < 3; ++j) v[3 * u + j] = ld<true>(&vp[(3 * tu + j) * 64]);
    }
  }
  T xq[NB][4];
  bool ok[NB];
#pragma unroll
  for (int u = 0; u < NB; ++u) {
    const int32_t c = d16_col(q[u], rowa, gb);
    ok[u] = c >= 0 && (FULL || t + u < ntri);
    x.quad(c >= 0 ? c : 0, xq[u]);
  }
#pragma unroll
  for (int u = 0; u < NB; ++u)
#pragma unroll
    for (int j = 0; j < 3; ++j) {
      const T t0 = acc[0] + term<ALPHA>(v[3 * u + j].v[0], xq[u][j], alpha, pf);
      const T t1 = acc[1] + term<ALPHA>(v[3 * u + j].v[1], xq[u][j + 1], alpha, pf);
      acc[0] = pick(ok[u], t0, acc[0]);
      acc[1] = pick(ok[u], t1, acc[1]);
    }
}

template <typename T, bool ALPHA, typename XS, bool TP>
__device__ __forceinline__ void rows_t16_pair(T (&acc)[2], const uint16_t* __restrict__ cs,
                                              const Pack<T, 2>* __restrict__ vp, int len, const XS& x, T alpha,
                                              bool pf, int32_t rowa, int32_t gb) {
  constexpr int B = sizeof(T) == 4 ? 9 : kTriBatch;
  const int ntri = len / 3;
  int t = 0;
  for (; t + B <= ntri; t += B) pair_batch<T, ALPHA, XS, TP, B, true>(acc, cs, vp, t, ntri, x, alpha, pf, rowa, gb, true);
  if constexpr (sizeof(T) == 4) {
    if (t < ntri) pair_batch<T, ALPHA, XS, TP, B, false>(acc, cs, vp, t, ntri, x, alpha, pf, rowa, gb, false);
  } else {
    for (; t < ntri; ++t) pair_batch<T, ALPHA, XS, TP, 1, true>(acc, cs, vp, t, ntri, x, alpha, pf, rowa, gb, false);
  }
}

template <typename T, int R, bool ALPHA, bool NT, int U, bool XP, bool SH = false, typename XS>
__device__ __forceinline__ void rows_pattern(T (&acc)[R], const int32_t* __restrict__ pat,
                                             const Pack<T, R>* __restrict__ vp, int len,
                                             const XS& x, int64_t rbase,
                                             const bool (&ok)[R], T alpha, bool pf, bool TB) {
  if (SH) TB = true;
  int64_t xb[R];
  bool any = false;
#pragma unroll
  for (int r = 0; r < R; ++r) {
    xb[r] = ok[r] ? rbase + r : -1;
    any = any || ok[r];
  }
  int k = 0;
  for (; !SH && k + U <= len; k += U) {
    int32_t o[U];
    Pack<T, R> v[U];
#pragma unroll
    for (int u = 0; u < U; ++u) o[u] = pat[k + u];
#pragma unroll
    for (int u = 0; u < U; ++u) v[u] = ld<NT>(&vp[(k + u) * 64]);
    T xv[U][R];
    if constexpr (XP && R > 1) {
#pragma unroll
      for (int u = 0; u < U; ++u) {
        const Pack<T, R> xr = x.template run<R>(any ? rbase + o[u] : 0);
#pragma unroll
        for (int r = 0; r < R; ++r) xv[u][r] = xr.v[r];
      }
    } else {
#pragma unroll
      for (int u = 0; u < U; ++u)
#pragma unroll
        for (int r = 0; r < R; ++r) xv[u][r] = x.get(xb[r] >= 0 ? xb[r] + o[u] : 0);
    }
#pragma unroll
    for (int u = 0; u < U; ++u)
#pragma unroll
      for (int r = 0; r < R; ++r) {
        acc[r] = acc[r] + term<ALPHA>(v[u].v[r], xv[u][r], alpha, pf);
      }
  }
  if (TB && k < len) {
    int32_t o[U];
    Pack<T, R> v[U];
#pragma unroll
    for (int u = 0; u < U; ++u) o[u] = pat[min(k + u, len - 1)];
#pragma unroll
    for (int u = 0; u < U; ++u)
      if (k + u < len) v[u] = ld<NT>(&vp[(k + u) * 64]);
    T xv[U][R];
    if constexpr (XP && R > 1) {
#pragma unroll
      for (int u = 0; u < U; ++u)
        if (k + u < len) {
          const Pack<T, R> xr = x.template run<R>(any ? rbase + o[u] : 0);
#pragma unroll
          for (int r = 0; r < R; ++r) xv[u][r] = xr.v[r];
        }
    } else {
#pragma unroll
      for (int u = 0; u < U; ++u)
        if (k + u < len)
#pragma unroll
          for (int r = 0; r < R; ++r) xv[u][r] = x.get(xb[r] >= 0 ? xb[r] + o[u] : 0);
    }
#pragma unroll
    for (int u = 0; u < U; ++u)
      if (k + u < len) {
#pragma unroll
        for (int r = 0; r < R; ++r) {
          acc[r] = acc[r] + term<ALPHA>(v[u].v[r], xv[u][r], alpha, pf);
        }
      }
    k = len;
  }
  for (; !SH && k < len; ++k) {
    const int32_t o = pat[k];
    const Pack<T, R> v = ld<NT>(&vp[k * 64]);
#pragma unroll
    for (int r = 0; r < R; ++r) {
      acc[r] = acc[r] + term<ALPHA>(v.v[r], x.get(xb[r] >= 0 ? xb[r] + o : 0), alpha, pf);
    }
  }
}

template <typename T, int R, bool ALPHA, bool NT, typename XS>
__device__ __forceinline__ void rows_pattern_tri(T (&acc)[R], const int32_t* __restrict__ pat,
                                                 const Pack<T, R>* __restrict__ vp, int len, const XS& x,
                                                 int64_t rbase, const bool (&ok)[R], T alpha, bool pf) {
  static_assert(R > 1, "runs of R > 1 values");
  bool any = false;
#pragma unroll
  for (int r = 0; r < R; ++r) any = any || ok[r];
  auto triple = [&](int32_t o, T (&xv)[3][R]) {
    Pack<T, R> A, B;
    if constexpr (R == 2 && sizeof(T) == 4) {
      T q[4];
      x.quad(any ? rbase + o : 0, q);
      A.v[0] = q[0];
      A.v[1] = q[1];
      B.v[0] = q[2];
      B.v[1] = q[3];
    } else {
      A = x.template run<R>(any ? rbase + o : 0);
      B = x.template run<R>(any ? rbase + o + 2 : 0);
    }
#pragma unroll
    for (int r = 0; r < R; ++r) {
      xv[0][r] = A.v[r];
      xv[1][r] = r + 1 < R ? A.v[r + 1] : B.v[R - 2];
      xv[2][r] = B.v[r];
    }
  };
  int k = 0;
  constexpr int TB = kTriBatch;
  for (; k + 3 * TB <= len; k += 3 * TB) {
    int32_t o[TB];
#pragma unroll
    for (int t = 0; t < TB; ++t) o[t] = pat[k + 3 * t];
    Pack<T, R> v[3 * TB];
#pragma unroll
    for (int u = 0; u < 3 * TB; ++u) v[u] = ld<NT>(&vp[(k + u) * 64]);
    T xv[TB][3][R];
#pragma unroll
    for (int t = 0; t < TB; ++t) triple(o[t], xv[t]);
#pragma unroll
    for (int t = 0; t < TB; ++t)
#pragma unroll
      for (int j = 0; j < 3; ++j)
#pragma unroll
        for (int r = 0; r < R; ++r) acc[r] = acc[r] + term<ALPHA>(v[3 * t + j].v[r], xv[t][j][r], alpha, pf);
  }
  for (; k < len; k += 3) {
    const int32_t o = pat[k];
    Pack<T, R> v[3];
#pragma unroll
    for (int j = 0; j < 3; ++j) v[j] = ld<NT>(&vp[(k + j) * 64]);
    T xv[3][R];
    triple(o, xv);
#pragma unroll
    for (int j = 0; j < 3; ++j)
#pragma unroll
      for (int r = 0; r < R; ++r) acc[r] = acc[r] + term<ALPHA>(v[j].v[r], xv[j][r], alpha, pf);
  }
}

template <typename W> __device__ inline W cg_alpha_of(const CGState* st);
template <> __device__ inline double cg_alpha_of<double>(const CGState* st) { return st->alpha.re; }
template <> __device__ inline c128 cg_alpha_of<c128>(const CGState* st) { return st->alpha; }

template <typename T, int R, bool UPD, typename XS, typename W>
__device__ __forceinline__ void cg_rows_update(const SpmvArgs<T>& a, const XS& xs, int64_t i0, int rs, W alpha,
                                               bool xpend = true, T* unv = nullptr) {
  T* xacc = (T*)a.xacc;
  T* un = (T*)a.un;
  if (rs == 1 && i0 + R <= a.nrows) {
    const Pack<T, R> uo = *reinterpret_cast<const Pack<T, R>*>(xs.u + i0);
    if (UPD) {
      const Pack<T, R> rv = *reinterpret_cast<const Pack<T, R>*>(xs.r + i0);
      Pack<T, R> o;
#pragma unroll
      for (int k = 0; k < R; ++k) o.v[k] = xs.f(rv.v[k], uo.v[k]);
      *reinterpret_cast<Pack<T, R>*>(un + i0) = o;
#pragma unroll
      for (int k = 0; k < R; ++k) unv[k] = o.v[k];
    }
    if (xpend) {
      Pack<T, R> xv = ld<true>(reinterpret_cast<const Pack<T, R>*>(xacc + i0));
#pragma unroll
      for (int k = 0; k < R; ++k) xv.v[k] = narrow<T>(widen(xv.v[k]) + alpha * widen(uo.v[k]));
      if constexpr (sizeof(Pack<T, R>) == 16) {
        spmv_u32x4 w;
        __builtin_memcpy(&w, &xv, 16);
        __builtin_nontemporal_store(w, reinterpret_cast<spmv_u32x4*>(xacc + i0));
      } else {
        *reinterpret_cast<Pack<T, R>*>(xacc + i0) = xv;
      }
    }
    return;
  }
#pragma unroll
  for (int k = 0; k < R; ++k) {
    const int64_t i = i0 + (int64_t)k * rs;
    if (i >= a.nrows) {
      if (UPD) unv[k] = zero_of<T>();
      continue;
    }
    const T uo = xs.u[i];
    if (UPD) {
      unv[k] = xs.f(xs.r[i], uo);
      un[i] = unv[k];
    }
    if (xpend) xacc[i] = narrow<T>(widen(xacc[i]) + alpha * widen(uo));
  }
}

template <typename T, int R, bool ALPHA, int BMODE, int U, int PK, bool SH = false, bool XV = false>
__device__ __forceinline__ void spmv_wave(const SpmvArgs<T>& a, const int64_t w) {
  constexpr bool PAT = PK == 1;
  constexpr int H = 64 * R;
  const int lane = threadIdx.x & 63;
  const int64_t s = a.list ? (int64_t)a.list[w] : w;
  bool il = false;
  if constexpr (PK == 3) il = kInterleaveD16<R>;
  if constexpr (PK == 4) il = true;
  if constexpr (PK == 0 && kInterleaveD16<R>) il = a.ilv && a.ilv[s] == kBkDelta16;
  const int rs = il ? 64 : 1;
  const int64_t row0 = s * H + (il ? (int64_t)lane : (int64_t)lane * R);
  XSrc<T, XV> xs;
  bool xpend = false, main_rows = false;
  typename wide_of<T>::type xalpha{};
  if constexpr (XV) {
    const CGState* cg = (const CGState*)a.cg;
    xpend = cg->it > cg->xit;
    xalpha = cg_alpha_of<typename wide_of<T>::type>(cg);
    xs.r = (const T*)a.x;
    xs.u = (const T*)a.xu;
    xs.b = (cg->res * cg->res) / (cg->prev * cg->prev);
    main_rows = a.rowmap == nullptr;
    if (cg->done) {
      if (xpend && main_rows) cg_rows_update<T, R, false>(a, xs, row0, rs, xalpha);
      return;
    }
  } else {
    xs.x = (const T*)a.x;
  }
  int64_t off;
  int32_t lraw;
  uint64_t dmask = 0;
  int32_t tgb = 0;
  if (PAT && a.desc) {
    constexpr int W = H / 64, DW = kDescWords<R>;
    typedef int iv __attribute__((ext_vector_type(DW)));
    const iv d = *reinterpret_cast<const iv*>(a.desc + DW * s);
    off = (int64_t)d[0] * H;
    lraw = d[1];
    const int wi = (lane * R) / 64;
#pragma unroll
    for (int i = 0; i < W; ++i) {
      const uint64_t mw = (uint64_t)(uint32_t)d[4 + 2 * i] | ((uint64_t)(uint32_t)d[5 + 2 * i] << 32);
      if (i == 0 || wi == i) dmask = mw;
    }
  } else if (PK == 4 && a.desc) {
    typedef int i4v __attribute__((ext_vector_type(4)));
    const i4v d = *reinterpret_cast<const i4v*>(a.desc + 4 * s);
    off = (int64_t)d[0] * H;
    lraw = d[1];
    tgb = d[2];
  } else {
    off = a.soff[s];
    lraw = a.slen[s];
  }
  const int len = PAT ? (lraw & 0xff) : (PK == 4 ? (lraw & kTriLen) : lraw);
  bool ok[R];
  if (PAT) {
    const uint64_t m = a.desc ? dmask : a.mask[s * (H / 64) + (lane * R) / 64];
#pragma unroll
    for (int r = 0; r < R; ++r) ok[r] = ((m >> ((lane * R + r) & 63)) & 1ull) && (row0 + r < a.nrows);
  } else {
#pragma unroll
    for (int r = 0; r < R; ++r) ok[r] = row0 + (int64_t)r * rs < a.nrows;
    if (a.sflags && a.sflags[s]) {
      const uint64_t m = a.lmask[s * (H / 64) + (lane * R) / 64];
#pragma unroll
      for (int r = 0; r < R; ++r) ok[r] = ok[r] && !((m >> ((lane * R + r) & 63)) & 1ull);
    }
  }
  int64_t orow[R];
#pragma unroll
  for (int r = 0; r < R; ++r) {
    const int64_t i = row0 + (int64_t)r * rs;
    orow[r] = ok[r] ? (a.rowmap ? (int64_t)a.rowmap[i] : i) : 0;
    if constexpr (PK == 4) {
      if (orow[r] < 0) {
        ok[r] = false;
        orow[r] = 0;
      }
    }
  }

  T acc[R];
#pragma unroll
  for (int r = 0; r < R; ++r) {
    if (BMODE == 0) {
      acc[r] = zero_of<T>();
    } else {
      T yo = zero_of<T>();
      if (ok[r]) yo = a.y[a.ymap ? (int64_t)a.ymap[orow[r]] : orow[r]];
      acc[r] = (BMODE == 2) ? yo * a.beta : yo;
    }
  }

  const Pack<T, R>* __restrict__ vp = reinterpret_cast<const Pack<T, R>*>(a.val + off) + lane;
  const bool tb = (a.flags & SPMV_TAILB) != 0;
  const bool pf = (a.flags & SPMV_PRODA) != 0;
  if constexpr (PK == 1) {
    const int32_t* pat = a.pat + (int64_t)(lraw >> 9) * a.kmax;
    bool tri_done = false;
    if constexpr (R > 1 && !SH) {
      if ((lraw & 0x100) && (a.flags & SPMV_XPAIR)) {
        if (a.flags & SPMV_NT) rows_pattern_tri<T, R, ALPHA, true>(acc, pat, vp, len, xs, row0, ok, a.alpha, pf);
        else rows_pattern_tri<T, R, ALPHA, false>(acc, pat, vp, len, xs, row0, ok, a.alpha, pf);
        tri_done = true;
      }
    }
    if (tri_done) {
    } else if (a.flags & SPMV_XPAIR) {
      if (a.flags & SPMV_NT) rows_pattern<T, R, ALPHA, true, U, true, SH>(acc, pat, vp, len, xs, row0, ok, a.alpha, pf, tb);
      else rows_pattern<T, R, ALPHA, false, U, true, SH>(acc, pat, vp, len, xs, row0, ok, a.alpha, pf, tb);
    } else {
      if (a.flags & SPMV_NT) rows_pattern<T, R, ALPHA, true, U, false, SH>(acc, pat, vp, len, xs, row0, ok, a.alpha, pf, tb);
      else rows_pattern<T, R, ALPHA, false, U, false, SH>(acc, pat, vp, len, xs, row0, ok, a.alpha, pf, tb);
    }
  } else if constexpr (PK == 3) {
    const S16Pack<R>* __restrict__ cp = reinterpret_cast<const S16Pack<R>*>(a.col16 + off) + lane;
    const int32_t gb = a.gbase[s];
    int32_t rw[R];
#pragma unroll
    for (int r = 0; r < R; ++r) rw[r] = (int32_t)row0 + r * kD16RowStride<R>;
    if (a.flags & SPMV_NT) rows_d16<T, R, ALPHA, true, U, SH, kIdsAhead<T, R>>(acc, cp, vp, len, xs, a.alpha, pf, tb, rw, gb);
    else rows_d16<T, R, ALPHA, false, U, SH, kIdsAhead<T, R>>(acc, cp, vp, len, xs, a.alpha, pf, tb, rw, gb);
  } else if constexpr (PK == 4) {
    const S16Pack<R>* __restrict__ cp = reinterpret_cast<const S16Pack<R>*>(a.col16 + off) + lane;
    const int32_t gb = a.desc ? tgb : a.gbase[s];
    int32_t rw[R];
#pragma unroll
    for (int r = 0; r < R; ++r) rw[r] = (int32_t)orow[r];
    if (lraw & kTriSlice) {
      bool packed = false;
      if constexpr (R == 2) {
        using XS = XSrc<T, XV>;
        const bool tp = sizeof(T) == 4 && (a.flags & SPMV_TPACK);
        packed = true;
        if (lraw & kTriPair) {
          const uint16_t* cs = (const uint16_t*)a.col16 + off;
          if constexpr (sizeof(T) == 4) {
            if (tp) rows_t16_pair<T, ALPHA, XS, true>(acc, cs, vp, len, xs, a.alpha, pf, rw[0], gb);
            else rows_t16_pair<T, ALPHA, XS, false>(acc, cs, vp, len, xs, a.alpha, pf, rw[0], gb);
          } else {
            rows_t16_pair<T, ALPHA, XS, false>(acc, cs, vp, len, xs, a.alpha, pf, rw[0], gb);
          }
        } else {
          packed = false;
        }
      }
      if (packed) {
      } else if (a.flags & SPMV_NT) rows_t16_tri<T, R, ALPHA, true>(acc, cp, vp, len, xs, a.alpha, pf, rw, gb);
      else rows_t16_tri<T, R, ALPHA, false>(acc, cp, vp, len, xs, a.alpha, pf, rw, gb);
    } else {
      if (a.flags & SPMV_NT) rows_d16<T, R, ALPHA, true, U, SH, kIdsAhead<T, R>>(acc, cp, vp, len, xs, a.alpha, pf, tb, rw, gb);
      else rows_d16<T, R, ALPHA, false, U, SH, kIdsAhead<T, R>>(acc, cp, vp, len, xs, a.alpha, pf, tb, rw, gb);
    }
  } else {
    const IPack<R>* __restrict__ cp = reinterpret_cast<const IPack<R>*>(a.col + off) + lane;
    if (a.flags & SPMV_NT) rows_int32<T, R, ALPHA, true, U, SH, kIdsAhead<T, R>>(acc, cp, vp, len, xs, a.alpha, pf, tb);
    else rows_int32<T, R, ALPHA, false, U, SH, kIdsAhead<T, R>>(acc, cp, vp, len, xs, a.alpha, pf, tb);
  }

  T un[R];
  if constexpr (XV) {
    if (main_rows) cg_rows_update<T, R, true>(a, xs, row0, rs, xalpha, xpend, un);
  }
  if (a.dotp) {
    using DA = typename DAcc<T>::type;
    DA part = zero_of<DA>();
#pragma unroll
    for (int r = 0; r < R; ++r) {
      T uv;
      if constexpr (XV) uv = main_rows ? un[r] : xs.get(orow[r]);
      else uv = a.dotu[orow[r]];
      if (ok[r]) part = part + dacc(cdot(uv, acc[r]));
    }
#pragma unroll
    for (int d = 32; d >= 1; d >>= 1) part = part + shfl_down_acc(part, d);
    if (lane == 0) reinterpret_cast<DA*>(a.dotp)[a.dot_base + s] = part;
  }

  bool all = true;
#pragma unroll
  for (int r = 0; r < R; ++r) all = all && ok[r];
  if (all && !a.ymap && !a.rowmap && !il) {
    Pack<T, R> o;
#pragma unroll
    for (int r = 0; r < R; ++r) o.v[r] = acc[r];
    if constexpr (sizeof(Pack<T, R>) == 16) {
      if (a.flags & SPMV_YNT) {
        spmv_u32x4 w;
        __builtin_memcpy(&w, &o, 16);
        __builtin_nontemporal_store(w, reinterpret_cast<spmv_u32x4*>(a.y + row0));
// ... 40 lines not shown
  for (int u = 0; u < U; ++u)
    if (u < K) v[u] = ld<true>(&vp[u * 64]);
  Pack<T, R> xr[U];
  const int64_t xmin = -(int64_t)(R - 1), xmax = a.nx - 1;
#pragma unroll
  for (int u = 0; u < U; ++u)
    if (u < K) {
      const int64_t j = row0 + a.upat[u];
      xr[u] = ld_xrun<T, R>((const T*)a.x + (j < xmin ? xmin : j > xmax ? xmax : j));
    }
  const int emask = d[2];
  uint64_t m = 0;
#pragma unroll
  for (int i = 0; i < H / 64; ++i) {
    const uint64_t mw = (uint64_t)(uint32_t)d[4 + 2 * i] | ((uint64_t)(uint32_t)d[5 + 2 * i] << 32);
    if (i == 0 || (lane * R) / 64 == i) m = mw;
  }
  bool ok[R];
#pragma unroll
  for (int r = 0; r < R; ++r) ok[r] = ((m >> ((lane * R + r) & 63)) & 1ull) && (row0 + r < a.nrows);
  T acc[R];
#pragma unroll
  for (int r = 0; r < R; ++r) {
    if (BMODE == 0) {
      acc[r] = zero_of<T>();
    } else {
      T yo = zero_of<T>();
      if (ok[r]) yo = a.y[a.ymap ? (int64_t)a.ymap[row0 + r] : row0 + r];
      acc[r] = (BMODE == 2) ? yo * a.beta : yo;
    }
  }
  const bool pf = (a.flags & SPMV_PRODA) != 0;
#pragma unroll
  for (int u = 0; u < U; ++u)
#pragma unroll
    for (int r = 0; r < R; ++r) {
      const T t = acc[r] + term<ALPHA>(v[u].v[r], xr[u].v[r], a.alpha, pf);
      acc[r] = pick(u < K && ((emask >> u) & 1), t, acc[r]);
    }
  if (a.dotp) {
    using DA = typename DAcc<T>::type;
    DA part = zero_of<DA>();
#pragma unroll
    for (int r = 0; r < R; ++r)
      if (ok[r]) part = part + dacc(cdot(a.dotu[row0 + r], acc[r]));
#pragma unroll
    for (int dd = 32; dd >= 1; dd >>= 1) part = part + shfl_down_acc(part, dd);
    if (lane == 0) reinterpret_cast<DA*>(a.dotp)[a.dot_base + s] = part;
  }
  bool all = true;
#pragma unroll
  for (int r = 0; r < R; ++r) all = all && ok[r];
  if (all && !a.ymap) {
    Pack<T, R> o;
#pragma unroll
    for (int r = 0; r < R; ++r) o.v[r] = acc[r];
    if constexpr (sizeof(Pack<T, R>) == 16) {
      if (a.flags & SPMV_YNT) {
        spmv_u32x4 yw;
        __builtin_memcpy(&yw, &o, 16);
        __builtin_nontemporal_store(yw, reinterpret_cast<spmv_u32x4*>(a.y + row0));
      } else {
        *reinterpret_cast<Pack<T, R>*>(a.y + row0) = o;
      }
    } else {
      *reinterpret_cast<Pack<T, R>*>(a.y + row0) = o;
    }
  } else {
#pragma unroll
    for (int r = 0; r < R; ++r)
      if (ok[r]) a.y[a.ymap ? (int64_t)a.ymap[row0 + r] : row0 + r] = acc[r];
  }
}

template <typename T>
struct SpmvGroup {
  int np;
  int tail0;
  int64_t start[PA_GROUP_MAX + 1];
  SpmvArgs<T> a[PA_GROUP_MAX];
};

template <typename T, int R, bool ALPHA, int BMODE, int U, int PK, bool SH = false, bool XV = false,
          bool TAIL = false>
__device__ __forceinline__ void group_wave(const SpmvGroup<T>& g) {
  const int64_t w = xcd_block(g.a[0].xcd_chunk) * 4 + __builtin_amdgcn_readfirstlane((int)(threadIdx.x >> 6));
  if (w >= g.start[g.np]) return;
  int p = 0;
  while (p + 1 < g.np && w >= g.start[p + 1]) ++p;
  p = __builtin_amdgcn_readfirstlane(p);
  if constexpr (TAIL) {
    if (p >= g.tail0) {
      spmv_wave<T, R, ALPHA, BMODE, 4, 0, false, false>(g.a[p], w - g.start[p]);
      return;
    }
  }
  if constexpr (PK == 1 && SH && !XV && U == 7) {
    if (g.a[p].uval) {
      spmv_wave_u<T, R, ALPHA, BMODE, U>(g.a[p], w - g.start[p]);
      return;
    }
  }
  spmv_wave<T, R, ALPHA, BMODE, U, PK, SH, XV>(g.a[p], w - g.start[p]);
}

template <typename T, int R, bool ALPHA, int BMODE, int U, int PK, bool SH = false, bool XV = false,
          bool TAIL = false>
__global__ __launch_bounds__(256) void k_spmv_sell_group(const SpmvGroup<T> g) {
  group_wave<T, R, ALPHA, BMODE, U, PK, SH, XV, TAIL>(g);
}

template <typename T, int R>
__global__ __launch_bounds__(256) __attribute__((amdgpu_waves_per_eu(7))) void k_spmv_group_short7(
    const SpmvGroup<T> g) {
  group_wave<T, R, false, 0, 7, 1, true, false, true>(g);
}

template <typename F>
static void with_ab(bool has_alpha, int bmode, F&& f) {
  auto with_b = [&](auto al) {
    if (bmode == 0) f(al, std::integral_constant<int, 0>{});
    else if (bmode == 1) f(al, std::integral_constant<int, 1>{});
    else f(al, std::integral_constant<int, 2>{});
  };
  if (has_alpha) with_b(std::true_type{});
  else with_b(std::false_type{});
}

template <int R, typename F>
static void with_pk(int pk, F&& f) {
  if (pk == kPkPattern) f(std::integral_constant<int, kPkPattern>{});
  else if (pk == kPkDelta16) f(std::integral_constant<int, kPkDelta16>{});
  else if (pk == kPkTriple) {
    if constexpr (R <= 2) f(std::integral_constant<int, kPkTriple>{});
  } else f(std::integral_constant<int, kPkInt32>{});
}

template <typename T, int R, bool ALPHA, int BMODE, int PAT>
static void launch_group_t(const SpmvGroup<T>& g, hipStream_t st) {
  const int64_t blocks = (g.start[g.np] + 3) / 4;
  if (blocks == 0) return;
  bool sh = (knobs().spmv_flags & SPMV_SHORT) != 0;
  for (int i = 0; i < g.np && i < g.tail0; ++i) sh = sh && g.a[i].maxlen <= 8;
  if constexpr (!ALPHA && BMODE == 0 && PAT != 4) {
    if (g.a[0].cg) {
      if (sh)
        hipLaunchKernelGGL((k_spmv_sell_group<T, R, false, 0, 8, PAT, true, true>), dim3(blocks), dim3(256), 0, st, g);
      else
        hipLaunchKernelGGL((k_spmv_sell_group<T, R, false, 0, 8, PAT, false, true>), dim3(blocks), dim3(256), 0, st, g);
      return;
    }
  }
  if constexpr (PAT == 1) {
    if (g.tail0 < g.np) {
      if constexpr (std::is_same<T, double>::value && !ALPHA && BMODE == 0) {
        bool sh7 = sh && (knobs().spmv_flags & SPMV_SHORT7) != 0 && knobs().spmv_xcd_chunk < 0;
        for (int i = 0; i < g.np && i < g.tail0; ++i) sh7 = sh7 && g.a[i].maxlen <= 7;
        if (sh7) {
          SpmvGroup<T> g2 = g;
          for (int i = 0; i < g2.np; ++i) g2.a[i].xcd_chunk = 0;
          hipLaunchKernelGGL((k_spmv_group_short7<T, R>), dim3(blocks), dim3(256), 0, st, g2);
          return;
        }
      }
      if (sh && knobs().spmv_xcd_chunk < 0) {
        SpmvGroup<T> g2 = g;
        for (int i = 0; i < g2.np; ++i) g2.a[i].xcd_chunk = 0;
        hipLaunchKernelGGL((k_spmv_sell_group<T, R, ALPHA, BMODE, 8, PAT, true, false, true>), dim3(blocks),
                           dim3(256), 0, st, g2);
      } else if (sh)
        hipLaunchKernelGGL((k_spmv_sell_group<T, R, ALPHA, BMODE, 8, PAT, true, false, true>), dim3(blocks),
                           dim3(256), 0, st, g);
      else
        hipLaunchKernelGGL((k_spmv_sell_group<T, R, ALPHA, BMODE, 8, PAT, false, false, true>), dim3(blocks),
                           dim3(256), 0, st, g);
      return;
    }
  }
  if (sh)
    hipLaunchKernelGGL((k_spmv_sell_group<T, R, ALPHA, BMODE, 8, PAT, true>), dim3(blocks), dim3(256), 0, st, g);
  else
    hipLaunchKernelGGL((k_spmv_sell_group<T, R, ALPHA, BMODE, 8, PAT>), dim3(blocks), dim3(256), 0, st, g);
}

template <typename T, int R, bool ALPHA, int BMODE, int PAT>
static void launch_t(const SpmvArgs<T>& a, hipStream_t st) {
  const int64_t blocks = (a.nwork + 3) / 4;
  if (blocks == 0) return;
  if constexpr (!ALPHA && BMODE == 0 && PAT != 4) {
    if (a.cg) {
      if ((knobs().spmv_flags & SPMV_SHORT) && a.maxlen <= 8)
        hipLaunchKernelGGL((k_spmv_sell<T, R, false, 0, 8, PAT, true, true>), dim3(blocks), dim3(256), 0, st, a);
      else
        hipLaunchKernelGGL((k_spmv_sell<T, R, false, 0, 8, PAT, false, true>), dim3(blocks), dim3(256), 0, st, a);
      return;
    }
  }
  if ((knobs().spmv_flags & SPMV_SHORT) && a.maxlen <= 8)
    hipLaunchKernelGGL((k_spmv_sell<T, R, ALPHA, BMODE, 8, PAT, true>), dim3(blocks), dim3(256), 0, st, a);
  else
    hipLaunchKernelGGL((k_spmv_sell<T, R, ALPHA, BMODE, 8, PAT>), dim3(blocks), dim3(256), 0, st, a);
}

struct KindDesc {
  const Sell* S;
  int pk;
  bool codes;
  bool idlist;
  int maxlen;
  const int32_t* slen;
  int64_t dot_base;
};

static KindDesc kind_desc(SliceKind k, const pa_mat* A) {
  const int64_t db = dot_base(A, k);
  switch (k) {
    case kPattern: return {&A->main, kPkPattern, false, true, A->maxlen_pat, A->d_plen, db};
    case kDelta16: return {&A->main, kPkDelta16, true, true, A->maxlen_d16, A->main.len, db};
    case kSide: return {&A->side, kPkInt32, false, false, A->side.maxlen, A->side.len, db};
    case kTriple:
      return {&A->tri, kPkTriple, true, false, std::max(A->tri.maxlen, 9), A->tri.len, db};
    case kInt32: break;
  }
  return {&A->main, kPkInt32, false, true, pattern_layout(A) ? A->maxlen_pm_int : A->main.maxlen, A->main.len, db};
}

template <typename T>
static SpmvArgs<T> make_args(SliceKind k, const SpmvPart& q, const void* alpha, const void* beta) {
  const pa_mat* A = q.A;
  const KindDesc d = kind_desc(k, A);
  SpmvArgs<T> a{};
  if (q.cg) {
    a.xu = (decltype(a.xu))((const T*)q.xu);
    a.un = (decltype(a.un))((T*)q.un);
    a.xacc = (decltype(a.xacc))((T*)q.xacc);
    a.cg = (decltype(a.cg))(q.cg);
  }
  a.dotu = (decltype(a.dotu))((const T*)q.x);
  a.dotp = q.dotp;
  a.dot_base = d.dot_base;
  a.nwork = q.nwork;
  const bool all = (knobs().spmv_flags & SPMV_IDLIST) && d.idlist && q.nwork == A->main.nslices;
  a.list = (decltype(a.list))(all ? nullptr : q.list);
  a.x = (decltype(a.x))((const T*)q.x);
  a.nx = A->ncols_lids;
  a.y = (decltype(a.y))((T*)q.y);
  a.ymap = (decltype(a.ymap))(q.ymap);
  a.alpha = *(const T*)alpha;
  a.beta = *(const T*)beta;
  a.flags = knobs().spmv_flags | (A->csr ? SPMV_PRODA : 0) | (k == kTriple && (A->tri.pack & 1) ? SPMV_TPACK : 0);
  a.xcd_chunk = knobs().spmv_xcd_chunk >= 0 ? knobs().spmv_xcd_chunk : A->xcd_auto;
  a.maxlen = d.maxlen;
  const Sell& S = *d.S;
  a.soff = (decltype(a.soff))(S.off.p);
  a.slen = (decltype(a.slen))(d.slen);
  a.col = (decltype(a.col))(S.col.p);
  a.col16 = (decltype(a.col16))(d.codes ? S.col16.p : nullptr);
  a.gbase = (decltype(a.gbase))(d.codes ? S.gbase.p : nullptr);
  a.val = (decltype(a.val))((const T*)S.val.p);
  a.rowmap = (decltype(a.rowmap))(S.rowmap.p);
  a.nrows = S.nrows;
  if (k == kTriple) {
    if (knobs().spmv_flags & SPMV_DESC) a.desc = (decltype(a.desc))(A->tri.desc.p);
  } else if (k == kPattern) {
    a.pat = (decltype(a.pat))(A->d_pat.p);
    a.mask = (decltype(a.mask))(A->d_mask.p);
    a.kmax = A->kmax;
    if (knobs().spmv_flags & SPMV_DESC) a.desc = (decltype(a.desc))(A->d_pdesc.p);
    if (A->uni.val && a.desc) {
      a.uval = (decltype(a.uval))((const T*)A->uni.val.p);
      a.uK = A->uni.K;
      for (int e = 0; e < 8; ++e) a.upat[e] = A->uni.pat[e];
    }
  } else if (k == kInt32) {
    a.sflags = (decltype(a.sflags))(A->d_sflags.p);
    a.lmask = (decltype(a.lmask))(A->d_lmask.p);
    if (A->main.col16 && A->R == 4 && !pattern_layout(A)) a.ilv = (decltype(a.ilv))(A->d_kind.p);
  }
  return a;
}

template <typename T, int R>
static void launch_which(SliceKind k, const SpmvPart& q, bool has_alpha, int bmode, const void* alpha,
                         const void* beta, hipStream_t st) {
  const SpmvArgs<T> a = make_args<T>(k, q, alpha, beta);
  with_pk<R>(kind_desc(k, q.A).pk, [&](auto pk) {
    with_ab(has_alpha, bmode, [&](auto al, auto bm) {
      launch_t<T, R, decltype(al)::value, decltype(bm)::value, decltype(pk)::value>(a, st);
    });
  });
}

template <typename T, int R>
static void group_which(SliceKind kind, int np, const SpmvPart* parts, bool has_alpha, int bmode, const void* alpha,
                        const void* beta, hipStream_t st) {
  SpmvGroup<T> g{};
  g.tail0 = PA_GROUP_MAX + 1;
  auto flush = [&]() {
    if (g.np == 0) return;
    with_pk<R>(kind_desc(kind, parts[0].A).pk, [&](auto pk) {
      with_ab(has_alpha, bmode, [&](auto al, auto bm) {
        launch_group_t<T, R, decltype(al)::value, decltype(bm)::value, decltype(pk)::value>(g, st);
      });
    });
    g = SpmvGroup<T>{};
    g.tail0 = PA_GROUP_MAX + 1;
  };
  for (int i = 0; i < np; ++i) {
    const SpmvPart& q = parts[i];
    if (q.nwork <= 0) continue;
    if (q.side && g.tail0 > g.np) g.tail0 = g.np;
    g.a[g.np] = make_args<T>(q.side ? kSide : kind, q, alpha, beta);
    g.start[g.np + 1] = g.start[g.np] + q.nwork;
    if (++g.np == PA_GROUP_MAX) flush();
  }
  flush();
}

#define PA_DT_DECL(k)                                                                                          \
  void spmv_group_##k(SliceKind kind, int np, const SpmvPart* parts, bool has_alpha, int bmode, const void* alpha,  \
                      const void* beta, hipStream_t st);                                                        \
  int spmv_merged_##k(int n, const SliceKind* kinds, const SpmvPart* parts, bool has_alpha, int bmode,      \
                      const void* alpha, const void* beta, pa_ctx* owner, hipStream_t st);                     \
  void spmv_long_##k(const pa_mat* A, const void* x, void* y, const int32_t* ymap, bool has_alpha, int bmode,  \
                     const void* alpha, const void* beta, void* dotp, int64_t dot_base, hipStream_t st);       \
  void spmv_part_##k(SliceKind kind, const SpmvPart& q, bool has_alpha, int bmode, const void* alpha,         \
                     const void* beta, hipStream_t st);
PA_DT_DECL(0)
PA_DT_DECL(1)
PA_DT_DECL(2)
PA_DT_DECL(3)
#undef PA_DT_DECL
#if defined(PA_SPMV_DT)
#if PA_SPMV_DT == 0
using DtT = float;
constexpr int kDtR = 4;
#elif PA_SPMV_DT == 1
using DtT = double;
constexpr int kDtR = 2;
#elif PA_SPMV_DT == 2
using DtT = c64;
constexpr int kDtR = 2;
#else
using DtT = c128;
constexpr int kDtR = 1;
#endif
constexpr bool kDtR2 = PA_SPMV_DT == 0;
void PA_CAT(spmv_group_, PA_SPMV_DT)(SliceKind kind, int np, const SpmvPart* parts, bool has_alpha, int bmode,
                                     const void* alpha, const void* beta, hipStream_t st) {
  if constexpr (kDtR2) {
    for (int i = 0; i < np;) {
      int j = i + 1;
      while (j < np && parts[j].A->R == parts[i].A->R) ++j;
      if (parts[i].A->R == 2) group_which<DtT, 2>(kind, j - i, parts + i, has_alpha, bmode, alpha, beta, st);
      else group_which<DtT, kDtR>(kind, j - i, parts + i, has_alpha, bmode, alpha, beta, st);
      i = j;
// ... 1047 lines not shown
  }
}

template <int R>
__device__ __forceinline__ int64_t main_slot0(int64_t soff, int w) {
  return kInterleaveD16<R> ? soff + (int64_t)(w & 63) * R + (w >> 6) : soff + (int64_t)(w / R) * R + (w % R);
}

template <int R>
__global__ void k_t_rowinfo(int64_t n, const int32_t* __restrict__ rows, int H, const int64_t* __restrict__ soff,
                            const int32_t* __restrict__ slen, const int32_t* __restrict__ col, int64_t noids,
                            int32_t* __restrict__ info) {
  const int64_t i = blockIdx.x * (int64_t)blockDim.x + threadIdx.x;
  if (i >= n) return;
  const int64_t row = rows[i], s = row / H;
  const int64_t b = main_slot0<R>(soff[s], (int)(row - s * H));
  const int L = slen[s];
  int len = 0;
  bool reg = true, ghost = false, pad = false, bad = false;
  int32_t prev = 0;
  for (int k = 0; k < L; ++k) {
    const int32_t c = col[b + (int64_t)k * 64 * R];
    if (c < 0) { pad = true; continue; }
    if (pad) bad = true;
    if (len % 3 != 0 && c != prev + 1) reg = false;
    ghost = ghost || c >= noids;
    prev = c;
    ++len;
  }
  reg = reg && len > 0 && len % 3 == 0;
  info[i] = len | (reg ? 1 << 28 : 0) | (ghost ? 1 << 29 : 0) | (bad ? 1 << 30 : 0);
}

template <int R>
__global__ void k_t_pairinfo(int64_t n, const int32_t* __restrict__ rows, int H, const int64_t* __restrict__ soff,
                             const int32_t* __restrict__ slen, const int32_t* __restrict__ col,
                             int32_t* __restrict__ pairable) {
  const int64_t i = blockIdx.x * (int64_t)blockDim.x + threadIdx.x;
  if (i >= n) return;
  int32_t ok = 0;
  if (i + 1 < n && rows[i + 1] == rows[i] + 1) {
    const int64_t ra = rows[i], rb = ra + 1, sa = ra / H, sb = rb / H;
    const int64_t ba = main_slot0<R>(soff[sa], (int)(ra - sa * H)), bb = main_slot0<R>(soff[sb], (int)(rb - sb * H));
    const int La = slen[sa], Lb = slen[sb];
    ok = 1;
    for (int k = 0; k < max(La, Lb); ++k) {
      const int32_t ca = k < La ? col[ba + (int64_t)k * 64 * R] : -1;
      const int32_t cb = k < Lb ? col[bb + (int64_t)k * 64 * R] : -1;
      if (ca < 0 && cb < 0) break;
      if (ca < 0 || cb != ca + 1) {
        ok = 0;
        break;
      }
    }
  }
  pairable[i] = ok;
}

template <typename E, int R>
__global__ void k_u_fill(int64_t ns, int H, int K, const int32_t* __restrict__ kind, const int64_t* __restrict__ soff,
                         const int32_t* __restrict__ plen, const int32_t* __restrict__ emap,
                         const E* __restrict__ val, E* __restrict__ uval) {
  const int64_t i = blockIdx.x * (int64_t)blockDim.x + threadIdx.x;
  if (i >= ns * 8 * 64) return;
  const int64_t s = i / (8 * 64);
  const int k = (int)((i / 64) % 8), l = (int)(i % 64);
  if (kind[s] != kBkPattern) return;
  const int32_t lraw = plen[s];
  if (k >= (lraw & 0xff)) return;
  const int e = emap[(lraw >> 9) * 8 + k];
#pragma unroll
  for (int r = 0; r < R; ++r)
    uval[s * H * K + ((int64_t)e * 64 + l) * R + r] = val[soff[s] + ((int64_t)k * 64 + l) * R + r];
}

void launch_u_fill(const pa_mat* A, hipStream_t st) {
  const int64_t n = A->main.nslices * 8 * 64;
  if (n == 0 || !A->uni.val) return;
  hipLaunchKernelGGL((k_u_fill<double, 2>), dim3((unsigned)((n + 255) / 256)), dim3(256), 0, st, A->main.nslices, A->H,
                     A->uni.K, A->d_kind, A->main.off, A->d_plen, A->uni.emap, (const double*)A->main.val,
                     (double*)A->uni.val);
}

void launch_t_pairinfo(const pa_mat* A, int64_t n, const int32_t* rows, int32_t* pairable, hipStream_t st) {
  if (n == 0) return;
  const dim3 g((unsigned)((n + 255) / 256)), b(256);
#define PA_TPI(RR) hipLaunchKernelGGL(k_t_pairinfo<RR>, g, b, 0, st, n, rows, A->H, A->main.off, A->main.len, \
                                      A->main.col, pairable)
  switch (A->R) {
    case 1: PA_TPI(1); break;
    case 2: PA_TPI(2); break;
    case 4: PA_TPI(4); break;
  }
#undef PA_TPI
}

template <int R>
__global__ __launch_bounds__(256) void k_t_gbase(int64_t ns, int64_t nrows, int H, const int32_t* __restrict__ rowlen,
                                                 const int64_t* __restrict__ src, const int32_t* __restrict__ col,
                                                 int64_t noids, int32_t* __restrict__ gbase, int32_t* __restrict__ ok) {
  const int64_t s = (int64_t)blockIdx.x * 4 + (threadIdx.x >> 6);
  if (s >= ns) return;
  const int lane = threadIdx.x & 63;
  int32_t gmin = INT32_MAX, gmax = -1;
  for (int w = lane; w < H; w += 64) {
    const int64_t i = s * H + w;
    if (i >= nrows) break;
    for (int k = 0; k < rowlen[i]; ++k) {
      const int32_t c = col[src[i] + (int64_t)k * 64 * R];
      if (c >= noids) { gmin = min(gmin, c); gmax = max(gmax, c); }
    }
  }
  for (int d = 32; d >= 1; d >>= 1) {
    gmin = min(gmin, __shfl_xor(gmin, d, 64));
    gmax = max(gmax, __shfl_xor(gmax, d, 64));
  }
  if (lane == 0) {
    gbase[s] = gmin == INT32_MAX ? 0 : gmin;
    ok[s] = gmin == INT32_MAX || (int64_t)gmax - gmin <= 32766;
  }
}

__device__ __forceinline__ int64_t t_code_slot(int64_t d, int g, int ntri, int lane, int r, int R, bool packed,
                                               int B) {
  const int b = g / B, i = g % B, nq = 4 * (B / 4);
  if (!packed || B * (b + 1) > ntri) return d + ((int64_t)g * 64 + lane) * R + r;
  const int64_t bb = d + (int64_t)b * B * 64 * R;
  return i < nq ? bb + (int64_t)(i / 4) * 4 * 64 * R + (int64_t)lane * 4 * R + (i % 4) * R + r
                : bb + (int64_t)i * 64 * R + (int64_t)lane * R + r;
}

template <typename E, int R>
__global__ void k_t_fill(int64_t nrows, int H, const int32_t* __restrict__ rowmap, const int32_t* __restrict__ rowlen,
                         const int64_t* __restrict__ src, const int64_t* __restrict__ toff,
                         const int32_t* __restrict__ tlen, const int32_t* __restrict__ gbase,
                         const int32_t* __restrict__ col, const E* __restrict__ val, int64_t noids, bool codes,
                         int pack, uint16_t* __restrict__ col16, E* __restrict__ tval) {
  const int64_t i = blockIdx.x * (int64_t)blockDim.x + threadIdx.x;
  if (i >= nrows) return;
  const int64_t ts = i / H;
  const int w = (int)(i - ts * H), lane = w & 63, r = w >> 6;
  if (rowmap[i] < 0) return;
  const int32_t lraw = tlen[ts];
  const int L = lraw & kTriLen;
  const bool tri = (lraw & kTriSlice) != 0, pair = (lraw & kTriPair) != 0;
  constexpr int B = sizeof(E) == 4 ? 9 : 4;
  const int n = rowlen[i];
  const int64_t b = src[i], d = toff[ts];
  const int32_t oid = rowmap[i], gb = gbase[ts];
  for (int k = 0; k < L; ++k) {
    const int64_t sk = b + (int64_t)k * 64 * R;
    E v;
    __builtin_memset(&v, 0, sizeof(E));
    if (k < n) v = val[sk];
    if ((pack & 1) && pair && sizeof(E) == 4) {
      const int64_t tb = d + (int64_t)(k / 3) * 3 * 64 * R;
      const int j = k % 3;
      tval[j < 2 ? tb + (int64_t)lane * 2 * R + j * R + r : tb + 2 * 64 * R + (int64_t)lane * R + r] = v;
    } else {
      tval[d + ((int64_t)k * 64 + lane) * R + r] = v;
    }
    if (!codes || (tri && k % 3 != 0) || (pair && r != 0)) continue;
    uint16_t q = 0xFFFFu;
    if (k < n) {
      const int32_t c = col[sk];
      q = c < noids ? (uint16_t)((uint32_t)(c - oid) & 0x7FFFu) : (uint16_t)(0x8000u | (uint32_t)(c - gb));
// ... 87 lines not shown
```

partitionedarrays.jl_amd/device.py:

```python
from __future__ import annotations

import ctypes as C
import sys

import numpy as np

from . import _lib
from .backends import DistributedBackend, PData, SequentialBackend


class PartContext:

    def __init__(self, device: int, part: int, nparts: int, share_with=None):
        h = C.c_void_p()
        if share_with is not None:
            _lib.call("pa_ctx_create_shared", part, nparts, share_with.h, C.byref(h))
        else:
            _lib.call("pa_ctx_create", device, part, nparts, C.byref(h))
        self.h = h
        self.device = device
        self.part = part
        self.nparts = nparts

    def sync(self):
# ... 587 lines not shown
        nzval = np.ascontiguousarray(nzval, dtype=self.dtype)
        _lib.call("pa_mat_set_values", self.h, nzval.ctypes.data_as(C.c_void_p))

    def fillstored(self, v):
        buf, ptr = _lib.scalar_buf(v, self.dtype)
        _lib.call("pa_mat_fillstored", self.h, ptr)
        del buf

    def get_values(self):
        n = getattr(self, "csc_nnz", None)
        if n is None:
            raise _lib.PAError("matrix was not built from a CSC pattern")
        a = np.empty(n, dtype=self.dtype)
        _lib.call("pa_mat_get_values", self.h, a.ctypes.data_as(C.c_void_p))
        return a

    def scatter(self, rows_idx: DeviceIndex, cols_idx: DeviceIndex, I, J, V, ids_global=False,
                op=_lib.PA_SCATTER_ADD):
        n, ib, on_device, (ip, jp), _ = _ids_args(ids_global, I, J)
        vp = _vals_arg(V, n, self.dtype, on_device)
        _lib.call("pa_mat_scatter", self.h, rows_idx.h, cols_idx.h,
                  _lib.PA_IDS_GLOBAL if ids_global else _lib.PA_IDS_LOCAL, ib, int(op), 1 if on_device else 0, n,
                  ip, jp, vp)

    def gather(self, rows_idx: DeviceIndex, cols_idx: DeviceIndex, I, J, ids_global=False, absent_zero=False,
               out=None):
        n, ib, on_device, (ip, jp), _ = _ids_args(ids_global, I, J)
        out, op = _out_arg(out, n, self.dtype, on_device)
        _lib.call("pa_mat_gather", self.h, rows_idx.h, cols_idx.h,
                  _lib.PA_IDS_GLOBAL if ids_global else _lib.PA_IDS_LOCAL, ib, 1 if absent_zero else 0,
                  1 if on_device else 0, n, ip, jp, op)
        return out

    def findnz(self, rows_idx: DeviceIndex, cols_idx: DeviceIndex, all_rows=False, ids_global=True) -> DeviceCOO:
        h = C.c_void_p()
        _lib.call("pa_mat_findnz", self.h, rows_idx.h, cols_idx.h,
                  _lib.PA_NZ_ALL_ROWS if all_rows else _lib.PA_NZ_OWNED_ROWS,
                  _lib.PA_IDS_GLOBAL if ids_global else _lib.PA_IDS_LOCAL, C.byref(h))
        return DeviceCOO._adopt(self.ctx, self.dtype, h)

    def entry_table(self):
        e, b = C.c_int64(), C.c_int64()
        _lib.call("pa_mat_entry_info", self.h, C.byref(e), C.byref(b))
        return e.value, b.value

    def cg_choice(self) -> int:
        v = C.c_int(-1)
        _lib.call("pa_mat_cg_choice", self.h, C.byref(v))
        return v.value

    def info(self):
        v = [C.c_int64() for _ in range(5)]
        _lib.call("pa_mat_info", self.h, *[C.byref(x) for x in v])
        d = dict(zip(["nrows", "nnz", "slots", "nslices", "nslices_interior"], [x.value for x in v]))
        f = [C.c_int64() for _ in range(4)]
        _lib.call("pa_mat_format_info", self.h, *[C.byref(x) for x in f])
        d.update(zip(["pattern_slices", "regular_rows", "side_rows", "side_slots"], [x.value for x in f]))
        dd = C.c_int64()
        _lib.call("pa_mat_delta16_info", self.h, C.byref(dd))
        d["delta16_slices"] = dd.value
        t = [C.c_int64() for _ in range(4)]
        _lib.call("pa_mat_triple_info", self.h, *[C.byref(x) for x in t])
        d.update(zip(["triple_sell_slices", "triple_sell_rows", "tri_slices", "tri_rows"], [x.value for x in t]))
        pr = [C.c_int64() for _ in range(2)]
        if hasattr(_lib.lib(), "pa_mat_pair_info"):
            _lib.call("pa_mat_pair_info", self.h, *[C.byref(x) for x in pr])
        d.update(zip(["pair_slices", "pair_rows"], [x.value for x in pr]))
        lr = [C.c_int64() for _ in range(2)]
        _lib.call("pa_mat_long_rows", self.h, *[C.byref(x) for x in lr])
        d.update(zip(["long_rows", "long_nnz"], [x.value for x in lr]))
        d.update(self.traffic())
        return d

    def device_ptrs(self):
        out = (C.c_uint64 * 8)()
        _lib.call("pa_mat_device_ptrs", self.h, out)
        return dict(zip(["val", "col", "slice_off", "plen", "pat", "mask", "s_val", "s_col"], list(out)))

    def traffic(self):
        t = [C.c_int64() for _ in range(3)]
        _lib.call("pa_mat_traffic", self.h, *[C.byref(x) for x in t])
        return dict(zip(["value_bytes", "index_bytes", "meta_bytes"], [x.value for x in t]))

    def __del__(self):
        try:
            if getattr(self, "h", None) and _lib._lib is not None and not sys.is_finalizing():
                _lib._lib.pa_mat_destroy(self.h)
        except Exception:
            pass
```

Measured before the change: 6795.

## Read one shared value row per pattern slice when all rows match

Adds a detection kernel that marks pattern slices whose valid rows all hold identical values, which is typical of constant-coefficient stencils. It also builds a compact per-slice value table. In the SpMV, those slices load their values once per wave through scalar (constant address space) loads instead of per-row vector loads, with a dedicated triple-run path. This is meant to remove most of the value-array HBM traffic. In exchange it costs extra setup work and a re-check whenever values change, plus a table allocation sized by slices times kmax. The short7 kernel path is excluded for such matrices.

```diff
diff --git a/include/pa_hip.h b/include/pa_hip.h
--- a/include/pa_hip.h
+++ b/include/pa_hip.h
@@ -190,6 +190,8 @@
 int pa_mat_traffic(const pa_mat* A, int64_t* value_bytes, int64_t* index_bytes,
                    int64_t* meta_bytes);
 
+int pa_mat_shared_info(const pa_mat* A, int64_t* shared_slices, int64_t* table_bytes);
+
 int pa_mat_long_rows(const pa_mat* A, int64_t* n_long, int64_t* n_long_nnz);
 
 int pa_spmv_all(int n, pa_mat* const A[], pa_vec* const y[],
diff --git a/partitionedarrays.jl_amd/_lib.py b/partitionedarrays.jl_amd/_lib.py
--- a/partitionedarrays.jl_amd/_lib.py
+++ b/partitionedarrays.jl_amd/_lib.py
@@ -156,6 +156,7 @@
     "pa_ctx_kernel_times": [_p, C.POINTER(C.c_float), C.POINTER(C.c_float), C.POINTER(C.c_float),
                             C.POINTER(C.c_int)],
     "pa_mat_traffic": [_p, _i64p, _i64p, _i64p],
+    "pa_mat_shared_info": [_p, _i64p, _i64p],
     "pa_mat_device_ptrs": [_p, _p],
     "pa_ctx_span": [_p, C.c_int],
     "pa_ctx_span_ms": [_p, C.POINTER(C.c_float)],
diff --git a/partitionedarrays.jl_amd/csrc/pa_api.cpp b/partitionedarrays.jl_amd/csrc/pa_api.cpp
--- a/partitionedarrays.jl_amd/csrc/pa_api.cpp
+++ b/partitionedarrays.jl_amd/csrc/pa_api.cpp
@@ -53,7 +53,7 @@
      65536,  2,  1,  0,  1,
      1,  0,  1,  0,  -1,  1,
      1,  1,  1,  0,  7,  1,
-     0};
+     0,  0};
 int coo_compress(int dtype, int index_bytes, int64_t m, int64_t ncols, int64_t n, const void* dI, const void* dJ,
                  const void* dV, int csr, int64_t* nu_out, DevBuf<int32_t>& crow, DevBuf<int32_t>& ccol,
                  DevBuf<void>& cval, DevBuf<int64_t>& colptr, hipStream_t st, hipError_t* err);
@@ -111,6 +111,7 @@
 void launch_t_rowinfo(const pa_mat* A, int64_t n, const int32_t* rows, int64_t noids, int32_t* info, hipStream_t st);
 void launch_t_pairinfo(const pa_mat* A, int64_t n, const int32_t* rows, int32_t* pairable, hipStream_t st);
 void launch_u_fill(const pa_mat* A, hipStream_t st);
+void launch_shr_detect(const pa_mat* A, hipStream_t st);
 void launch_t_gbase(const pa_mat* A, int64_t noids, int32_t* ok, hipStream_t st);
 void launch_t_fill(const pa_mat* A, int64_t noids, bool codes, hipStream_t st);
 void launch_t_check(const pa_mat* A, unsigned* bad, hipStream_t st);
@@ -720,6 +721,40 @@
   return 0;
 }
 
+int build_shared(pa_mat* A) {
+  A->shr = SharedRows{};
+  const int mode = knobs().spmv_share;
+  if (mode < 0 || A->uni.val || A->npattern_slices == 0) return 0;
+  const int64_t ns = A->main.nslices, S = (int64_t)dtype_size(A->dtype);
+  int64_t bytes = 0;
+  for (int64_t s = 0; s < ns; ++s)
+    if (A->h_kind[s] == kBkPattern) bytes += (int64_t)A->h_plen[s] * A->H * S;
+  if (mode == 0 && bytes <= kXcdL2Bytes) return 0;
+  hipStream_t st = A->ctx->s_main;
+  const size_t tb = (size_t)ns * A->kmax * S;
+  HIPC(A->shr.val.alloc(tb));
+  HIPC(hipMemsetAsync(A->shr.val, 0, tb, st));
+  launch_shr_detect(A, st);
+  HIPC(hipGetLastError());
+  HIPC(hipStreamSynchronize(st));
+  return 0;
+}
+
+int shared_flags(const pa_mat* A, std::vector<int32_t>* f) {
+  f->clear();
+  const bool desc_on = (knobs().spmv_flags & 2) != 0;
+  if (!A->shr.val || !desc_on || !pattern_layout(A)) return 0;
+  const int64_t ns = A->main.nslices;
+  const int DW = desc_words(A->R);
+  HIPC(hipSetDevice(A->ctx->device));
+  std::vector<int32_t> desc;
+  HIPC(download(desc, A->d_pdesc.p, (size_t)ns * DW, A->ctx->s_main));
+  HIPC(hipStreamSynchronize(A->ctx->s_main));
+  f->resize(ns);
+  for (int64_t s = 0; s < ns; ++s) (*f)[s] = desc[DW * s + kDescShared];
+  return 0;
+}
+
 int finalize_pattern(pa_mat* A, int kmax, int64_t noids, bool retry_r2) {
   A->kmax = std::max(kmax, 1);
   if (A->main.nslices == 0) return 0;
@@ -728,7 +763,7 @@
   if (retry_r2 && prefers_r2(A, D.kind)) return kPreferR2;
   std::vector<int32_t> kind = D.kind, side;
   if (dedup_patterns(A, kind) || encode_delta16(A, noids, kind) || build_slice_lists(A, kind, D, &side) ||
-      build_side_sell(A, side, noids))
+      build_side_sell(A, side, noids) || build_shared(A))
     return -1;
   A->has_pat = true;
   return 0;
@@ -1283,6 +1318,11 @@
     {"scatter_wide", &Knobs::scatter_wide, nullptr, 0, 1, 0,
      "scatter_wide: the ordered vector scatter (pa_vec_scatter) sorts 0 = 32-bit keys and payloads when the "
      "part's local ids and the entries fit them (default), 1 = always the 64-bit ones (A/B, tests)"},
+    {"spmv_share", &Knobs::spmv_share, nullptr, -1, 1, 0,
+     "spmv_share: pattern slices whose regular rows all hold the same values read one value row per slice "
+     "instead of one per row (matrices built afterwards; re-checked whenever the values change): 0 = auto "
+     "(default): matrices whose pattern slices hold more value bytes than one XCD's L2 (4 MiB), 1 = always, "
+     "-1 = never"},
     {"fault_inject", &Knobs::fault_inject, nullptr, 0, 1, 0,
      "fault_inject: 1 = every job of a threaded issue (IssuePool) also issues an invalid kernel launch (tests "
      "of the error path; test_exception.jl's role), 0 = off (default)"},
@@ -2823,6 +2863,10 @@
     launch_u_fill(A, st);
     HIPC(hipGetLastError());
   }
+  if (A->shr.val) {
+    launch_shr_detect(A, st);
+    HIPC(hipGetLastError());
+  }
   return 0;
 }
 
@@ -3065,9 +3109,14 @@
   const bool pat = pattern_layout(A);
   const bool split = A->sl_all.d_bnd != nullptr;
   int64_t v = 0, ix = 0, m = 0;
+  std::vector<int32_t> shf;
+  if (shared_flags(A, &shf)) return -1;
   for (int64_t s = 0; s < A->main.nslices; ++s) {
     const int kd = pat ? A->h_kind[s] : kBkInt32;
-    if (kd == kBkPattern) {
+    if (kd == kBkPattern && !shf.empty() && shf[s]) {
+      v += (int64_t)A->h_plen[s] * S;
+      m += std::max<int64_t>(W * 8 + 8 + 4, 4 * desc_words(A->R)) + 4;
+    } else if (kd == kBkPattern) {
       v += (int64_t)(A->uni.val ? A->uni.K : A->h_plen[s]) * H * S;
       m += std::max<int64_t>(W * 8 + 8 + 4, 4 * desc_words(A->R)) + 4;
     } else if (kd == kBkDelta16) {
@@ -3107,6 +3156,16 @@
   if (slots) *slots = A->main.slots;
   if (nslices) *nslices = A->main.nslices;
   if (nslices_int) *nslices_int = A->sl_all.n_int;
+  return 0;
+}
+
+int pa_mat_shared_info(const pa_mat* A, int64_t* shared_slices, int64_t* table_bytes) {
+  CHECK_ARG(A, "null matrix");
+  TuneScope ts(A->ctx);
+  std::vector<int32_t> shf;
+  if (shared_flags(A, &shf)) return -1;
+  if (shared_slices) *shared_slices = (int64_t)std::count_if(shf.begin(), shf.end(), [](int32_t f) { return f != 0; });
+  if (table_bytes) *table_bytes = A->shr.val ? A->main.nslices * A->kmax * (int64_t)dtype_size(A->dtype) : 0;
   return 0;
 }
 
diff --git a/partitionedarrays.jl_amd/csrc/pa_internal.h b/partitionedarrays.jl_amd/csrc/pa_internal.h
--- a/partitionedarrays.jl_amd/csrc/pa_internal.h
+++ b/partitionedarrays.jl_amd/csrc/pa_internal.h
@@ -319,6 +319,7 @@
   int tri_pack;
   int spmv_uniform;
   int scatter_wide;
+  int spmv_share;
 };
 const Knobs& knobs();
 struct KnobBind {
@@ -522,6 +523,11 @@
   int K = 0;
   int32_t pat[8] = {0, 0, 0, 0, 0, 0, 0, 0};
 };
+struct SharedRows {
+  DevBuf<void> val;
+};
+constexpr int kDescShared = 3;
+constexpr int64_t kXcdL2Bytes = 4 << 20;
 }
 
 struct pa_mat {
@@ -568,6 +574,7 @@
   pa::Sell side;
   pa::TripleSell tri;
   pa::UniformRows uni;
+  pa::SharedRows shr;
   pa::DevBuf<void> d_dotp;
 
   int64_t nrows_lids = 0;
diff --git a/partitionedarrays.jl_amd/csrc/pa_spmv.hip b/partitionedarrays.jl_amd/csrc/pa_spmv.hip
--- a/partitionedarrays.jl_amd/csrc/pa_spmv.hip
+++ b/partitionedarrays.jl_amd/csrc/pa_spmv.hip
@@ -46,6 +46,12 @@
 #define PA_GLB
 #endif
 
+#if defined(__HIP_DEVICE_COMPILE__)
+#define PA_CONST __attribute__((address_space(4)))
+#else
+#define PA_CONST
+#endif
+
 template <int BYTES> struct RawOf;
 template <> struct RawOf<2> { typedef unsigned short type; };
 template <> struct RawOf<4> { typedef unsigned int type; };
@@ -60,6 +66,22 @@
   else r = *reinterpret_cast<const Raw*>(p);
   V v;
   __builtin_memcpy(&v, &r, sizeof(V));
+  return v;
+}
+
+template <typename T>
+__device__ __forceinline__ const PA_CONST T* scalar_ptr(const T* p) {
+  const uint64_t v = (uint64_t)p;
+  const uint64_t u = (uint64_t)(uint32_t)__builtin_amdgcn_readfirstlane((int)(uint32_t)v) |
+                     ((uint64_t)(uint32_t)__builtin_amdgcn_readfirstlane((int)(uint32_t)(v >> 32)) << 32);
+  return (const PA_CONST T*)u;
+}
+template <typename T>
+__device__ __forceinline__ T ld_s(const PA_CONST T* p) {
+  typedef typename RawOf<sizeof(T)>::type Raw;
+  const Raw r = *reinterpret_cast<const PA_CONST Raw*>(p);
+  T v;
+  __builtin_memcpy(&v, &r, sizeof(T));
   return v;
 }
 
@@ -100,6 +122,7 @@
   const PA_GLB T* uval;
   int uK;
   int32_t upat[8];
+  const PA_GLB T* shr;
 };
 
 template <typename T> struct DAcc { using type = double; };
@@ -599,11 +622,25 @@
   }
 }
 
-template <typename T, int R, bool ALPHA, bool NT, int U, bool XP, bool SH = false, typename XS>
+template <bool NT, bool SV, typename T, int R>
+__device__ __forceinline__ Pack<T, R> ld_val(const Pack<T, R>* __restrict__ vp, const PA_CONST T* sv, int k) {
+  if constexpr (SV) {
+    const T t = ld_s(sv + k);
+    Pack<T, R> v;
+#pragma unroll
+    for (int r = 0; r < R; ++r) v.v[r] = t;
+    return v;
+  } else {
+    return ld<NT>(&vp[k * 64]);
+  }
+}
+
+template <typename T, int R, bool ALPHA, bool NT, int U, bool XP, bool SH = false, bool SV = false, typename XS>
 __device__ __forceinline__ void rows_pattern(T (&acc)[R], const int32_t* __restrict__ pat,
                                              const Pack<T, R>* __restrict__ vp, int len,
                                              const XS& x, int64_t rbase,
-                                             const bool (&ok)[R], T alpha, bool pf, bool TB) {
+                                             const bool (&ok)[R], T alpha, bool pf, bool TB,
+                                             const PA_CONST T* sv = nullptr) {
   if (SH) TB = true;
   int64_t xb[R];
   bool any = false;
@@ -619,7 +656,7 @@
 #pragma unroll
     for (int u = 0; u < U; ++u) o[u] = pat[k + u];
 #pragma unroll
-    for (int u = 0; u < U; ++u) v[u] = ld<NT>(&vp[(k + u) * 64]);
+    for (int u = 0; u < U; ++u) v[u] = ld_val<NT, SV>(vp, sv, k + u);
     T xv[U][R];
     if constexpr (XP && R > 1) {
 #pragma unroll
@@ -648,7 +685,7 @@
     for (int u = 0; u < U; ++u) o[u] = pat[min(k + u, len - 1)];
 #pragma unroll
     for (int u = 0; u < U; ++u)
-      if (k + u < len) v[u] = ld<NT>(&vp[(k + u) * 64]);
+      if (k + u < len) v[u] = ld_val<NT, SV>(vp, sv, k + u);
     T xv[U][R];
     if constexpr (XP && R > 1) {
 #pragma unroll
@@ -677,11 +714,33 @@
   }
   for (; !SH && k < len; ++k) {
     const int32_t o = pat[k];
-    const Pack<T, R> v = ld<NT>(&vp[k * 64]);
+    const Pack<T, R> v = ld_val<NT, SV>(vp, sv, k);
 #pragma unroll
     for (int r = 0; r < R; ++r) {
       acc[r] = acc[r] + term<ALPHA>(v.v[r], x.get(xb[r] >= 0 ? xb[r] + o : 0), alpha, pf);
     }
+  }
+}
+
+template <typename T, int R, typename XS>
+__device__ __forceinline__ void x_triple(const XS& x, bool any, int64_t j, T (&xv)[3][R]) {
+  Pack<T, R> A, B;
+  if constexpr (R == 2 && sizeof(T) == 4) {
+    T q[4];
+    x.quad(any ? j : 0, q);
+    A.v[0] = q[0];
+    A.v[1] = q[1];
+    B.v[0] = q[2];
+    B.v[1] = q[3];
+  } else {
+    A = x.template run<R>(any ? j : 0);
+    B = x.template run<R>(any ? j + 2 : 0);
+  }
+#pragma unroll
+  for (int r = 0; r < R; ++r) {
+    xv[0][r] = A.v[r];
+    xv[1][r] = r + 1 < R ? A.v[r + 1] : B.v[R - 2];
+    xv[2][r] = B.v[r];
   }
 }
 
@@ -693,26 +752,7 @@
   bool any = false;
 #pragma unroll
   for (int r = 0; r < R; ++r) any = any || ok[r];
-  auto triple = [&](int32_t o, T (&xv)[3][R]) {
-    Pack<T, R> A, B;
-    if constexpr (R == 2 && sizeof(T) == 4) {
-      T q[4];
-      x.quad(any ? rbase + o : 0, q);
-      A.v[0] = q[0];
-      A.v[1] = q[1];
-      B.v[0] = q[2];
-      B.v[1] = q[3];
-    } else {
-      A = x.template run<R>(any ? rbase + o : 0);
-      B = x.template run<R>(any ? rbase + o + 2 : 0);
-    }
-#pragma unroll
-    for (int r = 0; r < R; ++r) {
-      xv[0][r] = A.v[r];
-      xv[1][r] = r + 1 < R ? A.v[r + 1] : B.v[R - 2];
-      xv[2][r] = B.v[r];
-    }
-  };
+  auto triple = [&](int32_t o, T (&xv)[3][R]) { x_triple<T, R>(x, any, rbase + o, xv); };
   int k = 0;
   constexpr int TB = kTriBatch;
   for (; k + 3 * TB <= len; k += 3 * TB) {
@@ -744,6 +784,53 @@
 #pragma unroll
       for (int r = 0; r < R; ++r) acc[r] = acc[r] + term<ALPHA>(v[j].v[r], xv[j][r], alpha, pf);
   }
+}
+
+constexpr int kShareTri = 9, kShareVals = 3;
+template <typename T, int R, bool ALPHA, bool WIDE, typename XS>
+__device__ __forceinline__ void rows_pattern_tri_shared(T (&acc)[R], const PA_CONST int32_t* pat,
+                                                        const PA_CONST T* sv, int len, const XS& x,
+                                                        int64_t rbase, const bool (&ok)[R], T alpha, bool pf) {
+  static_assert(R > 1, "runs of R > 1 values");
+  bool any = false;
+#pragma unroll
+  for (int r = 0; r < R; ++r) any = any || ok[r];
+  int k = 0;
+  auto batch = [&](auto nb) {
+    constexpr int NB = decltype(nb)::value, VG = NB < kShareVals ? NB : kShareVals;
+    int32_t o[NB];
+#pragma unroll
+    for (int t = 0; t < NB; ++t) o[t] = ld_s(pat + k + 3 * t);
+    T xv[NB][3][R];
+#pragma unroll
+    for (int t = 0; t < NB; ++t) x_triple<T, R>(x, any, rbase + o[t], xv[t]);
+    constexpr int NG = (NB + VG - 1) / VG;
+    T v[2][3 * VG];
+    auto values = [&](int g) {
+#pragma unroll
+      for (int u = 0; u < 3 * VG; ++u)
+        if (3 * VG * g + u < 3 * NB) v[g & 1][u] = ld_s(sv + k + 3 * VG * g + u);
+    };
+    values(0);
+#pragma unroll
+    for (int g = 0; g < NG; ++g) {
+      if (g + 1 < NG) values(g + 1);
+#pragma unroll
+      for (int t = VG * g; t < VG * (g + 1) && t < NB; ++t)
+#pragma unroll
+        for (int j = 0; j < 3; ++j)
+#pragma unroll
+          for (int r = 0; r < R; ++r)
+            acc[r] = acc[r] + term<ALPHA>(v[g & 1][3 * (t - VG * g) + j], xv[t][j][r], alpha, pf);
+      if (g + 1 < NG) __builtin_amdgcn_sched_barrier(0);
+    }
+    k += 3 * NB;
+  };
+  if constexpr (WIDE) {
+    while (k + 3 * kShareTri <= len) batch(std::integral_constant<int, kShareTri>{});
+  }
+  while (k + 3 * kTriBatch <= len) batch(std::integral_constant<int, kTriBatch>{});
+  while (k < len) batch(std::integral_constant<int, 1>{});
 }
 
 template <typename W> __device__ inline W cg_alpha_of(const CGState* st);
@@ -796,7 +883,7 @@
   }
 }
 
-template <typename T, int R, bool ALPHA, int BMODE, int U, int PK, bool SH = false, bool XV = false>
+template <typename T, int R, bool ALPHA, int BMODE, int U, int PK, bool SH = false, bool XV = false, bool SHR = true>
 __device__ __forceinline__ void spmv_wave(const SpmvArgs<T>& a, const int64_t w) {
   constexpr bool PAT = PK == 1;
   constexpr int H = 64 * R;
@@ -830,12 +917,14 @@
   int32_t lraw;
   uint64_t dmask = 0;
   int32_t tgb = 0;
+  bool shared = false;
   if (PAT && a.desc) {
     constexpr int W = H / 64, DW = kDescWords<R>;
     typedef int iv __attribute__((ext_vector_type(DW)));
     const iv d = *reinterpret_cast<const iv*>(a.desc + DW * s);
     off = (int64_t)d[0] * H;
     lraw = d[1];
+    if constexpr (SHR) shared = a.shr && __builtin_amdgcn_readfirstlane(d[kDescShared]) != 0;
     const int wi = (lane * R) / 64;
 #pragma unroll
     for (int i = 0; i < W; ++i) {
@@ -897,15 +986,23 @@
   const bool pf = (a.flags & SPMV_PRODA) != 0;
   if constexpr (PK == 1) {
     const int32_t* pat = a.pat + (int64_t)(lraw >> 9) * a.kmax;
-    bool tri_done = false;
-    if constexpr (R > 1 && !SH) {
-      if ((lraw & 0x100) && (a.flags & SPMV_XPAIR)) {
+    bool tri = false;
+    if constexpr (R > 1 && !SH) tri = (lraw & 0x100) && (a.flags & SPMV_XPAIR);
+    if (shared) {
+      const PA_CONST T* sv = scalar_ptr((const T*)a.shr + s * a.kmax);
+      if (tri) {
+        if constexpr (R > 1 && !SH)
+          rows_pattern_tri_shared<T, R, ALPHA, !ALPHA && !XV>(acc, scalar_ptr(pat), sv, len, xs, row0, ok, a.alpha, pf);
+      } else if (a.flags & SPMV_XPAIR) {
+        rows_pattern<T, R, ALPHA, false, U, true, SH, true>(acc, pat, vp, len, xs, row0, ok, a.alpha, pf, tb, sv);
+      } else {
+        rows_pattern<T, R, ALPHA, false, U, false, SH, true>(acc, pat, vp, len, xs, row0, ok, a.alpha, pf, tb, sv);
+      }
+    } else if (tri) {
+      if constexpr (R > 1 && !SH) {
         if (a.flags & SPMV_NT) rows_pattern_tri<T, R, ALPHA, true>(acc, pat, vp, len, xs, row0, ok, a.alpha, pf);
         else rows_pattern_tri<T, R, ALPHA, false>(acc, pat, vp, len, xs, row0, ok, a.alpha, pf);
-        tri_done = true;
-      }
-    }
-    if (tri_done) {
+      }
     } else if (a.flags & SPMV_XPAIR) {
       if (a.flags & SPMV_NT) rows_pattern<T, R, ALPHA, true, U, true, SH>(acc, pat, vp, len, xs, row0, ok, a.alpha, pf, tb);
       else rows_pattern<T, R, ALPHA, false, U, true, SH>(acc, pat, vp, len, xs, row0, ok, a.alpha, pf, tb);
@@ -1112,7 +1209,7 @@
 };
 
 template <typename T, int R, bool ALPHA, int BMODE, int U, int PK, bool SH = false, bool XV = false,
-          bool TAIL = false>
+          bool TAIL = false, bool SHR = true>
 __device__ __forceinline__ void group_wave(const SpmvGroup<T>& g) {
   const int64_t w = xcd_block(g.a[0].xcd_chunk) * 4 + __builtin_amdgcn_readfirstlane((int)(threadIdx.x >> 6));
   if (w >= g.start[g.np]) return;
@@ -1131,7 +1228,7 @@
       return;
     }
   }
-  spmv_wave<T, R, ALPHA, BMODE, U, PK, SH, XV>(g.a[p], w - g.start[p]);
+  spmv_wave<T, R, ALPHA, BMODE, U, PK, SH, XV, SHR>(g.a[p], w - g.start[p]);
 }
 
 template <typename T, int R, bool ALPHA, int BMODE, int U, int PK, bool SH = false, bool XV = false,
@@ -1143,7 +1240,7 @@
 template <typename T, int R>
 __global__ __launch_bounds__(256) __attribute__((amdgpu_waves_per_eu(7))) void k_spmv_group_short7(
     const SpmvGroup<T> g) {
-  group_wave<T, R, false, 0, 7, 1, true, false, true>(g);
+  group_wave<T, R, false, 0, 7, 1, true, false, true, false>(g);
 }
 
 template <typename F>
@@ -1185,7 +1282,7 @@
     if (g.tail0 < g.np) {
       if constexpr (std::is_same<T, double>::value && !ALPHA && BMODE == 0) {
         bool sh7 = sh && (knobs().spmv_flags & SPMV_SHORT7) != 0 && knobs().spmv_xcd_chunk < 0;
-        for (int i = 0; i < g.np && i < g.tail0; ++i) sh7 = sh7 && g.a[i].maxlen <= 7;
+        for (int i = 0; i < g.np && i < g.tail0; ++i) sh7 = sh7 && g.a[i].maxlen <= 7 && !g.a[i].shr;
         if (sh7) {
           SpmvGroup<T> g2 = g;
           for (int i = 0; i < g2.np; ++i) g2.a[i].xcd_chunk = 0;
@@ -1302,6 +1399,7 @@
       a.uK = A->uni.K;
       for (int e = 0; e < 8; ++e) a.upat[e] = A->uni.pat[e];
     }
+    if (A->shr.val && a.desc) a.shr = (decltype(a.shr))((const T*)A->shr.val.p);
   } else if (k == kInt32) {
     a.sflags = (decltype(a.sflags))(A->d_sflags.p);
     a.lmask = (decltype(a.lmask))(A->d_lmask.p);
@@ -2515,6 +2613,70 @@
                      (double*)A->uni.val);
 }
 
+template <int DWE, int R>
+__global__ __launch_bounds__(256) void k_shr_detect(int64_t ns, int64_t nrows, int kmax,
+                                                    const int32_t* __restrict__ kind,
+                                                    const int64_t* __restrict__ soff,
+                                                    const int32_t* __restrict__ plen,
+                                                    const uint64_t* __restrict__ mask,
+                                                    const uint32_t* __restrict__ val, uint32_t* __restrict__ sval,
+                                                    int32_t* __restrict__ desc) {
+  constexpr int H = 64 * R, DW = desc_words(R);
+  const int lane = threadIdx.x & 63;
+  const int64_t s = (int64_t)blockIdx.x * 4 + (threadIdx.x >> 6);
+  if (s >= ns) return;
+  bool shared = false;
+  if (kind[s] == kBkPattern) {
+    const int len = plen[s] & 0xff;
+    const uint64_t m = mask[s * (H / 64) + (lane * R) / 64];
+    bool ok[R];
+    int r0 = R;
+#pragma unroll
+    for (int r = R - 1; r >= 0; --r) {
+      ok[r] = ((m >> ((lane * R + r) & 63)) & 1ull) && s * H + (int64_t)lane * R + r < nrows;
+      if (ok[r]) r0 = r;
+    }
+    const unsigned long long have = __ballot(r0 < R);
+    if (have) {
+      const int fl = __ffsll(have) - 1;
+      const int fr = __shfl(r0, fl, 64);
+      const int64_t base = soff[s];
+      bool agree = true;
+      for (int k = 0; k < len; ++k) {
+        const uint32_t* ref = val + (base + ((int64_t)k * 64 + fl) * R + fr) * DWE;
+#pragma unroll
+        for (int r = 0; r < R; ++r) {
+          const uint32_t* p = val + (base + ((int64_t)k * 64 + lane) * R + r) * DWE;
+#pragma unroll
+          for (int d = 0; d < DWE; ++d) agree = agree && (!ok[r] || p[d] == ref[d]);
+        }
+        if (lane < DWE) sval[(s * kmax + k) * DWE + lane] = ref[lane];
+      }
+      shared = __all(agree);
+    }
+  }
+  if (lane == 0) desc[DW * s + kDescShared] = shared ? 1 : 0;
+}
+
+void launch_shr_detect(const pa_mat* A, hipStream_t st) {
+  const int64_t ns = A->main.nslices;
+  if (ns == 0 || !A->shr.val) return;
+  const dim3 g((unsigned)((ns + 3) / 4)), b(256);
+#define PA_SHR(DWE, RR) hipLaunchKernelGGL((k_shr_detect<DWE, RR>), g, b, 0, st, ns, A->main.nrows, A->kmax, A->d_kind, \
+                                           A->main.off, A->d_plen, A->d_mask, (const uint32_t*)A->main.val,            \
+                                           (uint32_t*)A->shr.val, A->d_pdesc)
+  switch (A->dtype) {
+    case PA_F32:
+      if (A->R == 4) PA_SHR(1, 4);
+      else PA_SHR(1, 2);
+      break;
+    case PA_F64: PA_SHR(2, 2); break;
+    case PA_C64: PA_SHR(2, 2); break;
+    case PA_C128: PA_SHR(4, 1); break;
+  }
+#undef PA_SHR
+}
+
 void launch_t_pairinfo(const pa_mat* A, int64_t n, const int32_t* rows, int32_t* pairable, hipStream_t st) {
   if (n == 0) return;
   const dim3 g((unsigned)((n + 255) / 256)), b(256);
diff --git a/partitionedarrays.jl_amd/device.py b/partitionedarrays.jl_amd/device.py
--- a/partitionedarrays.jl_amd/device.py
+++ b/partitionedarrays.jl_amd/device.py
@@ -693,6 +693,11 @@
         _lib.call("pa_mat_traffic", self.h, *[C.byref(x) for x in t])
         return dict(zip(["value_bytes", "index_bytes", "meta_bytes"], [x.value for x in t]))
 
+    def shared_info(self):
+        t = [C.c_int64() for _ in range(2)]
+        _lib.call("pa_mat_shared_info", self.h, *[C.byref(x) for x in t])
+        return dict(zip(["shared_slices", "table_bytes"], [x.value for x in t]))
+
     def __del__(self):
         try:
             if getattr(self, "h", None) and _lib._lib is not None and not sys.is_finalizing():
```

Result: slower. 2070 (-69.5%).
